# zhaoyizhou1123/OfflineRL-Kit

Measured on AMD Instinct MI355X. Metric: gradient-steps/sec (CQL, batch=256), higher is better.
Workload: dtype f32 storage / accumulate; products on split-fp16 MFMA (every operand = fp16 hi + fp16 lo plane = 22 significand bits, power-of-two operand scales folded back into the fp32 accumulators, hi*hi + hi*lo + lo*hi on v_mfma_f32_16x16x32_f16; the reference's fp32 has 24): losses and Q-values meet the 1e-4

## Files before the change

offlinerl-kit_amd/csrc/gemm.h:

```cpp
#pragma once
#include <hip/hip_runtime.h>
#include <stdint.h>

#include <algorithm>
#include <atomic>

namespace orl {

typedef float f32x4 __attribute__((ext_vector_type(4)));

#ifdef ORL_SPLIT_BF16
typedef __bf16 hx_t;
#define ORL_SPLIT_BITS 16
#define ORL_HX_ONE_BITS 0x3F80u
#define ORL_MFMA_16x16x32(a, b, c) __builtin_amdgcn_mfma_f32_16x16x32_bf16(a, b, c, 0, 0, 0)
#else
typedef _Float16 hx_t;
#define ORL_SPLIT_BITS 22
#define ORL_HX_ONE_BITS 0x3C00u
#define ORL_MFMA_16x16x32(a, b, c) __builtin_amdgcn_mfma_f32_16x16x32_f16(a, b, c, 0, 0, 0)
#endif
typedef hx_t hx4 __attribute__((ext_vector_type(4)));
typedef hx_t hx8 __attribute__((ext_vector_type(8)));
#define ORL_WSCALE 64.0f
#define ORL_WWSCALE 256.0f
#define ORL_GSCALE3 32.0f

#if defined(__HIP_DEVICE_COMPILE__) || defined(__HIPCC__)
typedef unsigned int u32x2_t __attribute__((ext_vector_type(2)));
typedef short s16x4 __attribute__((ext_vector_type(4)));
#ifdef ORL_SPLIT_BF16
#define ORL_MFMA_16x16x16(a, b, c) __builtin_amdgcn_mfma_f32_16x16x16bf16_1k(a, b, c, 0, 0, 0)
__device__ __forceinline__ void orl_split4(const f32x4& v, hx4& h, hx4& l) {
  h = __builtin_convertvector(v, hx4);
  const u32x2_t hb = *(const u32x2_t*)&h;
  f32x4 hf;
  hf[0] = __uint_as_float(hb[0] << 16); hf[1] = __uint_as_float(hb[0] & 0xffff0000u);
  hf[2] = __uint_as_float(hb[1] << 16); hf[3] = __uint_as_float(hb[1] & 0xffff0000u);
  l = __builtin_convertvector(v - hf, hx4);
}
#else
typedef _Float16 f16x4_t __attribute__((ext_vector_type(4)));
#define ORL_MFMA_16x16x16(a, b, c) __builtin_amdgcn_mfma_f32_16x16x16f16(*(const f16x4_t*)&(a), *(const f16x4_t*)&(b), c, 0, 0, 0)
__device__ __forceinline__ void orl_split4(const f32x4& v, hx4& h, hx4& l) {
  h = __builtin_convertvector(v, hx4);
#ifdef ORL_SPLIT_NO_MIX
  l = __builtin_convertvector(v - __builtin_convertvector(h, f32x4), hx4);
  return;
#endif
  const u32x2_t hb = *(const u32x2_t*)&h;
  f32x4 r;
  asm("v_fma_mix_f32 %0, %1, -1.0, %2 op_sel_hi:[1,0,0]" : "=v"(r[0]) : "v"(hb[0]), "v"(v[0]));
  asm("v_fma_mix_f32 %0, %1, -1.0, %2 op_sel:[1,0,0] op_sel_hi:[1,0,0]" : "=v"(r[1]) : "v"(hb[0]), "v"(v[1]));
  asm("v_fma_mix_f32 %0, %1, -1.0, %2 op_sel_hi:[1,0,0]" : "=v"(r[2]) : "v"(hb[1]), "v"(v[2]));
  asm("v_fma_mix_f32 %0, %1, -1.0, %2 op_sel:[1,0,0] op_sel_hi:[1,0,0]" : "=v"(r[3]) : "v"(hb[1]), "v"(v[3]));
  l = __builtin_convertvector(r, hx4);
}
#endif
__device__ __forceinline__ void orl_split1(float x, hx_t& h, hx_t& l) { h = (hx_t)x; l = (hx_t)(x - (float)h); }
__device__ __forceinline__ void orl_split4x3(const f32x4& v, hx4& h, hx4& m, hx4& l) {
  h = __builtin_convertvector(v, hx4);
#if defined(ORL_SPLIT_BF16) || defined(ORL_SPLIT_NO_MIX)
  const f32x4 r1 = v - __builtin_convertvector(h, f32x4);
  m = __builtin_convertvector(r1, hx4);
  l = __builtin_convertvector(r1 - __builtin_convertvector(m, f32x4), hx4);
#else
  const u32x2_t hb = *(const u32x2_t*)&h;
  f32x4 r1, r2;
  asm("v_fma_mix_f32 %0, %1, -1.0, %2 op_sel_hi:[1,0,0]" : "=v"(r1[0]) : "v"(hb[0]), "v"(v[0]));
  asm("v_fma_mix_f32 %0, %1, -1.0, %2 op_sel:[1,0,0] op_sel_hi:[1,0,0]" : "=v"(r1[1]) : "v"(hb[0]), "v"(v[1]));
  asm("v_fma_mix_f32 %0, %1, -1.0, %2 op_sel_hi:[1,0,0]" : "=v"(r1[2]) : "v"(hb[1]), "v"(v[2]));
  asm("v_fma_mix_f32 %0, %1, -1.0, %2 op_sel:[1,0,0] op_sel_hi:[1,0,0]" : "=v"(r1[3]) : "v"(hb[1]), "v"(v[3]));
  m = __builtin_convertvector(r1, hx4);
  const u32x2_t mb = *(const u32x2_t*)&m;
  asm("v_fma_mix_f32 %0, %1, -1.0, %2 op_sel_hi:[1,0,0]" : "=v"(r2[0]) : "v"(mb[0]), "v"(r1[0]));
  asm("v_fma_mix_f32 %0, %1, -1.0, %2 op_sel:[1,0,0] op_sel_hi:[1,0,0]" : "=v"(r2[1]) : "v"(mb[0]), "v"(r1[1]));
  asm("v_fma_mix_f32 %0, %1, -1.0, %2 op_sel_hi:[1,0,0]" : "=v"(r2[2]) : "v"(mb[1]), "v"(r1[2]));
  asm("v_fma_mix_f32 %0, %1, -1.0, %2 op_sel:[1,0,0] op_sel_hi:[1,0,0]" : "=v"(r2[3]) : "v"(mb[1]), "v"(r1[3]));
  l = __builtin_convertvector(r2, hx4);
#endif
}
__device__ __forceinline__ void orl_split1x3(float x, hx_t& h, hx_t& m, hx_t& l) {
  h = (hx_t)x;
  const float r1 = x - (float)h;
  m = (hx_t)r1;
  l = (hx_t)(r1 - (float)m);
}
__device__ __forceinline__ unsigned int orl_relu_mask4(f32x4& z) {
  unsigned int m = 0;
#pragma unroll
  for (int j = 0; j < 4; ++j) {
    const int r = max(__float_as_int(z[j]), 0);
    z[j] = __int_as_float(r);
    unsigned int b;
    asm("v_min_u32 %0, 1, %1" : "=v"(b) : "v"(r));
    m |= b << j;
  }
  return m;
}
__device__ __forceinline__ unsigned int orl_mask4(const f32x4& z) {
  unsigned int m = 0;
#pragma unroll
  for (int j = 0; j < 4; ++j) {
    const int b = min(max(__float_as_int(z[j]), 0), 1);
    m |= (unsigned int)b << j;
  }
  return m;
}
#endif

enum { P_F32 = 0, P_SPLIT = 1, P_BF16X3 = P_SPLIT, P_SPLIT3 = 2 };

enum { PA_PLAIN = 0, PA_RANK1 = 1, PA_RANK1B = 2 };
typedef unsigned int u32x4 __attribute__((ext_vector_type(4)));
enum { PB_PLAIN = 0, PB_ONES = 1 };
enum { E_PLAIN = 0, E_BIAS = 1, E_BIAS_RELU = 2, E_MASK = 3, E_WGRAD = 4,
       E_BIAS_SWISH = 5,
       E_SWISH_GRAD = 6,
       E_BIAS_LEAKY = 7,
       E_LEAKY_MASK = 8 };
#define ORL_LEAKY_SLOPE 0.01f
enum { L_SCALAR = 0, L_VECK = 1, L_BLK4 = 2, L_VECKU = 3 };

template <typename T>
struct ZView {
  T* p;
  long s0, s1;
  __host__ __device__ T* at(int z0, int z1) const { return p ? p + z0 * s0 + z1 * s1 : nullptr; }
  bool vec4() const { return (((uintptr_t)p) & 15) == 0 && !(s0 & 3) && !(s1 & 3); }
};
using ZPtr = ZView<const float>;
using ZOut = ZView<float>;
using ZBits = ZView<unsigned int>;

struct GemmP {
  ZPtr A, B;
  float* C;
  long c_s0, c_s1;
  long c_sr;
  long c_sn;
  long c_ks;
  int M, N, K;
  long a_sr, a_sk;
  long b_sr, b_sk;
  int a_rlim, b_rlim;
  int nz1;
  int ksplit;
  ZPtr rowv, colv;
  int a_trans;
  int ones_row;
  ZPtr bias;
  ZPtr aux;
  long aux_sr;
  float* bias_out;
  long bo_s0, bo_s1, bo_ks;
  float* tail_w_out; float* tail_b_out;
  long tw_s0, tw_s1, tb_s1;
  ZPtr tq_w, tq_b; float* tq_out; float* tq_part; long tq_s0, tq_s1, tq_sm, tq_ps0, tq_ps1, tq_ts;
  unsigned int* mb_out; long mb_s0, mb_s1; int mb_g;
  const unsigned int* aux_bits; long xb_s0, xb_s1; int xb_g;
  const unsigned int* a_bits; long ab_s0, ab_s1; int ab_g;
  ZPtr w0_x; long w0_xsr; int w0_in;
  float* w0_out; float* w0_bias; long w0_s0, w0_s1, w0_bs1, w0_ks, w0_sr;
  float a_scale, b_scale;
  const float* a_dscale; const float* b_dscale;
  int zmajor, nz_total;
  float* z_out;
};

#if defined(__HIP_DEVICE_COMPILE__) || defined(__HIPCC__)
__device__ __forceinline__ float orl_sigmoid(float z) { return __frcp_rn(1.0f + __expf(-z)); }
__device__ __forceinline__ float orl_swish(float z) { return z * orl_sigmoid(z); }
__device__ __forceinline__ float orl_dswish(float z) { const float s = orl_sigmoid(z); return s * (1.0f + z * (1.0f - s)); }
#endif

enum { W0_XP = 28 };

template <int WM, int WN, int MA, int NB, int TK>
struct GemmCfg {
  static constexpr int kWM = WM, kWN = WN, kMA = MA, kNB = NB, kTK = TK;
  static constexpr int TM = WM * MA * 16, TN = WN * NB * 16, NT = WM * WN * 64, PITCH = TK + 4;
  static constexpr int PITCH_H = TK + 8;
  static constexpr int LDS_FLOATS = 2 * (TM + TN) * PITCH;
  static constexpr size_t lds_bytes(int prec) {
    return prec == P_F32 ? sizeof(float) * LDS_FLOATS : (size_t)2  * (prec == P_SPLIT3 ? 3 : 2)  * (TM + TN) * PITCH_H * 2;
  }
  static constexpr size_t epi_lds_limit(int prec) { return lds_bytes(prec) > 80 * 1024 ? (size_t)160 * 1024 : lds_bytes(prec); }
  static constexpr size_t epi_lds_bytes() { return sizeof(float) * (size_t)TM * (TN + 4); }
  static_assert(TK % 16 == 0, "TK multiple of 16");
};

typedef GemmCfg<2, 4, 2, 4, 32> CfgBig;
typedef GemmCfg<2, 2, 2, 2, 32> CfgMid;
typedef GemmCfg<1, 4, 1, 1, 64> CfgSmall;
typedef GemmCfg<4, 1, 1, 1, 32> CfgTall;
typedef GemmCfg<2, 2, 4, 4, 32> CfgSq;
typedef GemmCfg<2, 4, 4, 2, 32> CfgSq8;
typedef GemmCfg<4, 2, 4, 4, 32> CfgWg;
enum { CFG_BIG = 0, CFG_MID = 1, CFG_SMALL = 2, CFG_TALL = 3, CFG_SQ = 4, CFG_SQ8 = 5, CFG_WG = 6, CFG_AUTO = -1 };

static inline int pick_cfg(int M, int N, int K, int nz) {
  if (N <= 16) return CFG_TALL;
  if (M >= 2048 && N >= 128) return ((long)M * nz >= 40000) ? CFG_SQ : CFG_BIG;
  if (M <= 32) return CFG_SMALL;
  if (K < 1024 && M >= 64 && N > 16 && N < 64 && (long)nz * ((M + 63) / 64) >= 1024) return CFG_MID;
  if (K < 1024 && M >= 64 && N >= 64) {
    if (K <= 32 && M >= 128 && N >= 128 && (long)nz * ((M + 127) / 128) * ((N + 127) / 128) >= 1024) return CFG_SQ;
    if (K >= 256 && M >= 128 && N >= 128 && (long)nz * ((M + 127) / 128) * ((N + 127) / 128) >= 256) return CFG_SQ;
    if ((long)nz * ((M + 63) / 64) * ((N + 63) / 64) >= 1024) return CFG_MID;
  }
  if (K >= 1024) return (M >= 256 && N >= 128) ? CFG_WG : ((M >= 128 && N >= 128) ? CFG_SQ : CFG_MID);
  return CFG_SMALL;
}

static inline bool aligned16(const void* p) { return (((uintptr_t)p) & 15) == 0; }

static inline int tq_fused_parts(int cfg, const GemmP& p, const float* tail_w, long tw_s0, long tw_s1) {
  const int TN = cfg == CFG_SQ8 ? CfgSq8::TN : (cfg == CFG_BIG ? CfgBig::TN : 0);
  if (!TN) return 0;
  if ((p.N & 3) || !aligned16(p.C) || (p.c_sr & 3) || (p.c_s0 & 3) || (p.c_s1 & 3) || p.c_sn != 1) return 0;
  if (!aligned16(p.bias.p) || (p.bias.s0 & 3) || (p.bias.s1 & 3)) return 0;
  if (!aligned16(tail_w) || (tw_s0 & 3) || (tw_s1 & 3)) return 0;
  return (p.N + TN - 1) / TN;
}

static inline bool mb_supported(int cfg, const GemmP& p) {
  if (cfg == CFG_TALL || (p.N & 31)) return false;
  if (!aligned16(p.C) || (p.c_sr & 3) || (p.c_s0 & 3) || (p.c_s1 & 3) || p.c_sn != 1) return false;
  return aligned16(p.bias.p) && !(p.bias.s0 & 3) && !(p.bias.s1 & 3);
}

static inline int w0_fused_slabs(const GemmP& p, int nz, int in0, long x_pitch, const void* x_ptr, long x_s0, long x_s1, int max_slab) {
  const int cfg = pick_cfg(p.M, p.N, p.K, nz);
  const int TM = cfg == CFG_SQ ? CfgSq::TM : (cfg == CFG_BIG ? CfgBig::TM : 0);
  if (!TM) return 0;
  if (in0 + 1 > W0_XP || in0 >= x_pitch || x_pitch > W0_XP || (x_pitch & 3) || !aligned16(x_ptr) || (x_s0 & 3) || (x_s1 & 3)) return 0;
  if (p.N & 3) return 0;
  if (!p.aux_bits && ((p.aux_sr & 3) || !aligned16(p.aux.p) || (p.aux.s0 & 3) || (p.aux.s1 & 3))) return 0;
  if (p.C && (!aligned16(p.C) || (p.c_sr & 3) || (p.c_s0 & 3) || (p.c_s1 & 3) || p.c_sn != 1)) return 0;
  const int tiles_m = (p.M + TM - 1) / TM;
  return tiles_m <= max_slab ? tiles_m : 0;
}

static inline int pick_loader(const ZPtr& z, long sr, long sk, int K, bool k_pad_ok, int rlim) {
  if (sk == 1 && (!aligned16(z.p) || (z.s0 & 3) || (z.s1 & 3) || (sr & 3) || !((K & 3) == 0 || k_pad_ok))) return L_VECKU;
  if (!aligned16(z.p) || (z.s0 & 3) || (z.s1 & 3)) return L_SCALAR;
  if (sk == 1 && (sr & 3) == 0 && ((K & 3) == 0 || k_pad_ok)) return L_VECK;
  if (sr == 1 && (sk & 3) == 0 && rlim >= 4 && (rlim & 3) == 0) return L_BLK4;
  return L_SCALAR;
}

static inline bool rank1_wgrad_is_fast(const GemmP& p, bool force_scalar) {
  if (force_scalar || p.a_trans != 1) return false;
  if (pick_loader(p.A, p.a_sr, p.a_sk, p.K, false, p.a_rlim) != L_BLK4) return false;
  if (pick_loader(p.B, p.b_sr, p.b_sk, p.K, false, p.b_rlim) != L_BLK4) return false;
  return aligned16(p.colv.p) && (p.colv.s0 & 3) == 0 && (p.colv.s1 & 3) == 0;
}

static inline bool rank1_bits_supported(int cfg, const GemmP& p, bool force_scalar) {
  if (force_scalar || (cfg != CFG_SQ && cfg != CFG_BIG) || p.a_trans != 0 || (p.K & 31)) return false;
  if (!aligned16(p.colv.p) || (p.colv.s0 & 3) || (p.colv.s1 & 3)) return false;
  const int lb = pick_loader(p.B, p.b_sr, p.b_sk, p.K, false, p.b_rlim);
  return lb == L_BLK4 || lb == L_VECK;
}

template <int PA, int PB, int EPI>
hipError_t launch_gemm(int cfg, const GemmP& p, int nz, hipStream_t st, bool a_kpad = false, bool force_scalar = false, int prec = P_F32);
template <int EPI>
hipError_t launch_gemm_rank1_bits(int cfg, const GemmP& p, int nz, hipStream_t st, int prec);
hipError_t launch_tune(int cfg_in, int kind, const GemmP& p, int nz, hipStream_t st);

}
```

offlinerl-kit_amd/csrc/ws_debug.hip:

```cpp
#include <hip/hip_runtime.h>

#include <cstring>
#include <string>
#include <vector>

#include "../../include/orl_engine.h"
#include "ws_gemm.h"

namespace orl {

int fail(const std::string& msg);

namespace {

typedef const WsTable& (*WsTableFn)();
static const WsTableFn WS_TABLES[] = {ws_fwd_table, ws_fwd3_table, ws_dgrad_table, ws_dgrad3_table, ws_wgrad_table, ws_wgrad3p_table};

struct WsDev {
  std::vector<void*> ptrs;
  ~WsDev() { for (void* q : ptrs) hipFree(q); }
};

enum { B_X, B_W, B_BIAS, B_TW, B_TB, B_X0, B_W0, B_B0, B_DMASK, B_ABITS, B_XBITS, B_DQ, B_WT, B_Z, B_H0, B_H1, B_W1, B_B1, B_DZ, B_GSCALE,
       B_Y, B_MB, B_MB0, B_TQ, B_TQ2, B_C, B_W0O, B_B0O, B_DW, B_DB, B_DWT, B_DBT, B_COUNT };
static const char* const WS_BUF_NAMES[B_COUNT] = {"X", "W", "bias", "tw", "tb", "X0", "W0", "b0", "dmask", "abits", "xbits", "dq", "wt", "Z", "H0", "H1",
                                                   "W1", "b1", "dZ", "gscale", "Y", "mb", "mb0", "tq", "tq2", "C", "w0_out", "b0_out", "dW", "db", "dwt", "dbt"};

static bool ws_buf_allowed(int kind, int i) {
  const bool fwd = kind == ORL_WS_FWD || kind == ORL_WS_FWD3, dg = kind == ORL_WS_DGRAD || kind == ORL_WS_DGRAD3;
  switch (i) {
    case B_X: case B_W: return fwd || dg;
    case B_BIAS: case B_TW: case B_TB: case B_DMASK: case B_Y: case B_MB: case B_MB0: case B_TQ: return fwd;
    case B_TQ2: return kind == ORL_WS_FWD3;
    case B_X0: case B_W0: case B_B0: return fwd || kind == ORL_WS_WGRAD;
    case B_XBITS: case B_Z: case B_C: case B_W0O: case B_B0O: return dg;
    case B_ABITS: case B_DQ: case B_WT: return dg || kind == ORL_WS_WGRAD;
    case B_H0: case B_DZ: case B_DW: case B_DB: return kind == ORL_WS_WGRAD || kind == ORL_WS_WGRAD3P;
    case B_H1: case B_W1: case B_B1: case B_DWT: case B_DBT: return kind == ORL_WS_WGRAD;
    default: return true;
  }
}

}
}

using namespace orl;

extern "C" {

const char* orl_debug_ws_flavour(int idx) {
  for (WsTableFn table : WS_TABLES) {
    const WsTable& t = table();
    if (idx >= 0 && idx < t.n) return t.rows[idx].name;
    idx -= t.n;
  }
  return nullptr;
}

int orl_debug_ws(orl_ws_ex* a) {
  if (!a) return fail("orl_debug_ws: null arguments");
  const int kind = a->kind, M = a->M, nz0 = a->nz0, nz1 = a->nz1, per_z = a->per_z;
  auto bad = [](const std::string& m) { return fail("orl_debug_ws: " + m); };
  if (kind < ORL_WS_FWD || kind > ORL_WS_WGRAD3P) return bad("kind must be 0..5");
  if (M < 1 || M > 4096) return bad("M must be 1..4096");
  if (M % WS_ROWS) return bad("M must be a multiple of 32 (whole row groups)");
  if (nz0 < 1 || nz1 < 1 || (long)nz0 * nz1 > 64) return bad("nz0 x nz1 must be 1..64");
  if (per_z < 1) return bad("per_z must be >= 1");
  if (per_z > M / WS_ROWS) return bad("per_z exceeds the row groups (M / 32): a workgroup would own no group");
  const int nz = nz0 * nz1, groups = M / WS_ROWS;
  const bool fwd = kind == ORL_WS_FWD || kind == ORL_WS_FWD3, dg = kind == ORL_WS_DGRAD || kind == ORL_WS_DGRAD3;
  const bool wg = kind == ORL_WS_WGRAD || kind == ORL_WS_WGRAD3P;
  if (a->f32 && (kind == ORL_WS_FWD3 || kind == ORL_WS_DGRAD3 || kind == ORL_WS_WGRAD3P)) return bad("f32 does not go with a three-plane launcher");
  if (a->np3 && kind != ORL_WS_WGRAD) return bad("np3 selects ws_wgrad_kernel<5> of launch_ws_wgrad and nothing else");
  if (a->np3 && a->f32) return bad("np3 and f32 exclude each other");

  orl_gemm_buf* bufs[B_COUNT] = {&a->X, &a->W, &a->bias, &a->tw, &a->tb, &a->X0, &a->W0, &a->b0, &a->dmask, &a->abits, &a->xbits, &a->dq, &a->wt, &a->Z,
                                 &a->H0, &a->H1, &a->W1, &a->b1, &a->dZ, &a->gscale, &a->Y, &a->mb, &a->mb0, &a->tq, &a->tq2, &a->C, &a->w0_out, &a->b0_out,
                                 &a->dW, &a->db, &a->dwt, &a->dbt};
  auto has = [&](int i) { return bufs[i]->host != nullptr; };
  for (int i = 0; i < B_COUNT; ++i)
    if (has(i) && !ws_buf_allowed(kind, i)) return bad(std::string(WS_BUF_NAMES[i]) + " does not belong to this launcher");

  std::string why;
  auto fits = [&](int i, long ext, int nslab, bool result) {
    const orl_gemm_buf& b = *bufs[i];
    const std::string name = WS_BUF_NAMES[i];
    if (!b.host) { why = name + " is required"; return false; }
    if (b.n <= 0 || b.n > (1L << 28)) { why = name + ": bad element count"; return false; }
    if (b.off < 0 || b.s0 < 0 || b.s1 < 0 || b.ks < 0 || b.pitch < 0) { why = name + ": negative offset, pitch or stride"; return false; }
    if (ext < 1) { why = name + ": empty extent"; return false; }
    if (result && ((nz0 > 1 && b.s0 < ext) || (nz1 > 1 && b.s1 < ext) || (nslab > 1 && b.ks < ext))) { why = name + ": problems or slabs of a result overlap"; return false; }
    const long last = b.off + (long)(nz0 - 1) * b.s0 + (long)(nz1 - 1) * b.s1 + (long)(nslab - 1) * b.ks + ext;
    if (last > b.n) { why = name + ": the array is shorter than its offset, strides and pitch need"; return false; }
    return true;
  };
  auto rows_fit = [&](int i, long cols, bool result) {
    if (has(i) && bufs[i]->pitch < cols) { why = std::string(WS_BUF_NAMES[i]) + ": the pitch is below the width"; return false; }
    return fits(i, (long)(M - 1) * bufs[i]->pitch + cols, 1, result);
  };
  auto narrow_fit = [&](int i) {
    if (has(i) && (bufs[i]->pitch < 1 || bufs[i]->pitch > 32)) { why = std::string(WS_BUF_NAMES[i]) + ": the pitch must be 1..32"; return false; }
    return fits(i, (long)M * bufs[i]->pitch, 1, false);
  };
  auto strided_fit = [&](int i, long sn, long sk, int nn, int nk, int nslab, bool result) {
    if (sn < 1 || sk < 1) { why = std::string(WS_BUF_NAMES[i]) + ": strides must be >= 1"; return false; }
    return fits(i, (long)(nn - 1) * sn + (long)(nk - 1) * sk + 1, nslab, result);
  };
  const bool l0 = fwd && has(B_X0), recomp = wg && has(B_X0);
  if ((l0 || recomp || (dg && has(B_W0O))) && (a->in0 < 1 || a->in0 + 1 > 32)) return bad("in0 must be 1..31 (in0 + 1 <= 32: the ones column takes a slot)");
  if (has(B_GSCALE)) {
    const orl_gemm_buf& b = a->gscale;
    if (b.n <= 0 || b.off < 0 || b.off + nz0 > b.n) return bad("gscale: one float per run (nz0) from its offset");
  }

  if (fwd) {
    const bool dgm = has(B_DMASK), tq = has(B_TQ), sy = has(B_Y);
    if (a->tq_sm < 1) return bad("tq_sm must be >= 1");
    if (has(B_TW) != tq || has(B_TB) != tq) return bad("the fused tail needs tw, tb and tq together");
    if (kind == ORL_WS_FWD3 && tq && !has(B_TQ2)) return bad("the three-plane forward writes its tail as two partial sums: tq needs tq2");
    if (has(B_TQ2) && !tq) return bad("tq2 goes with tq");
    if (dgm && (tq || l0 || has(B_BIAS) || has(B_MB) || has(B_MB0))) return bad("plain dgrad mode (dmask) has no bias, tail, fused first layer or mask output");
    if (dgm && bufs[B_DMASK]->pitch != 8) return bad("dm_g (dmask's pitch) must be 8 words");
    if (l0 != has(B_W0) || l0 != has(B_B0) || l0 != has(B_MB0)) return bad("the fused first layer needs X0, W0, b0 and mb0 together");
    if (a->x0_discard && !l0) return bad("x0_discard belongs to the fused first layer");
    if (!rows_fit(B_X, WS_K, l0) || !strided_fit(B_W, a->w_sn, a->w_sk, WS_N, WS_K, 1, false)) return bad(why);
    if (!dgm && !has(B_MB)) return bad("mb is required (the forward always emits mask words)");
    if (!dgm && (!fits(B_BIAS, WS_N, 1, false) || !rows_fit(B_MB, 8, true))) return bad(why);
    if (sy && !rows_fit(B_Y, WS_N, true)) return bad(why);
    if (tq && (!fits(B_TW, WS_N, 1, false) || !fits(B_TB, 1, 1, false) || !fits(B_TQ, (long)(M - 1) * a->tq_sm + 1, 1, true))) return bad(why);
    if (has(B_TQ2) && !fits(B_TQ2, M, 1, true)) return bad(why);
    if (dgm && !rows_fit(B_DMASK, 8, false)) return bad(why);
    if (l0) {
      if (a->in0 >= bufs[B_X0]->pitch) return bad("in0 must be below x0_pitch (the ones column needs a slot of the staged row)");
      if (bufs[B_MB0]->pitch != 8) return bad("mb0_g (mb0's pitch) must be 8 words");
      if (!narrow_fit(B_X0) || !strided_fit(B_W0, a->w0_sn, a->w0_sk, WS_N, a->in0, 1, false) || !fits(B_B0, WS_N, 1, false) || !rows_fit(B_MB0, 8, true)) return bad(why);
    }
  } else if (dg) {
    const bool plain = has(B_Z), w0 = has(B_W0O), store = has(B_C);
    if (a->dq_sm < 1) return bad("dq_sm must be >= 1");
    if (w0 == store) return bad("give either the dW0 / db0 slabs (w0_out, b0_out) or C (the stored dz0), not both and not neither");
    if (w0 != has(B_B0O)) return bad("w0_out and b0_out go together");
    if (plain && (has(B_ABITS) || has(B_DQ) || has(B_WT))) return bad("the plain flavour (Z) takes no abits, dq or wt");
    if (!has(B_XBITS) || bufs[B_XBITS]->pitch != 8) return bad("xb_g (xbits' pitch) must be 8 words");
    if (!plain && (!has(B_ABITS) || bufs[B_ABITS]->pitch != 8)) return bad("ab_g (abits' pitch) must be 8 words");
    if (!rows_fit(B_XBITS, 8, false) || !strided_fit(B_W, a->w_sn, a->w_sk, WS_N, WS_K, 1, false)) return bad(why);
    if (plain) { if (!rows_fit(B_Z, WS_K, false)) return bad(why); }
    else if (!rows_fit(B_ABITS, 8, false) || !fits(B_DQ, (long)(M - 1) * a->dq_sm + 1, 1, false) || !fits(B_WT, WS_K, 1, false)) return bad(why);
    if (w0) {
      if (!has(B_X)) return bad("X is required");
      if (a->in0 >= bufs[B_X]->pitch) return bad("in0 must be below x_pitch (the ones column needs a slot of the staged row)");
      if (a->b0_out.s0 != a->w0_out.s0 || a->b0_out.ks != a->w0_out.ks) return bad("b0_out shares w0_out's s0 and slab stride");
      if (!narrow_fit(B_X) || !strided_fit(B_W0O, a->o_sr, a->o_sc, WS_N, a->in0, per_z, true) || !fits(B_B0O, WS_N, per_z, true)) return bad(why);
    } else {
      if (has(B_X)) return bad("X belongs to the dW0 / db0 flavour");
      if (!rows_fit(B_C, WS_N, true)) return bad(why);
    }
  } else {
    const bool plain = has(B_DZ), tails = has(B_H1), derived = !tails && has(B_W1);
    if (a->dq_sm < 1) return bad("dq_sm must be >= 1");
    if (kind == ORL_WS_WGRAD3P && !plain) return bad("launch_ws_wgrad3p is the plain (materialised dZ) flavour: dZ is required");
    if (a->np3 && tails) return bad("np3 is the derived-tail flavour: it takes W1 / b1, not H1");
    if (plain && (has(B_ABITS) || has(B_DQ) || has(B_WT) || tails || has(B_W1) || has(B_B1) || has(B_DWT) || has(B_DBT))) return bad("the plain flavour (dZ) takes no abits, dq, wt, H1, W1, b1 and writes no tail gradients");
    if (recomp && !plain) return bad("X0 (recompute) belongs to the plain flavour");
    if (recomp == has(B_H0)) return bad("give either H0 or X0 / W0 / b0 (recompute)");
    if (recomp != has(B_W0) || recomp != has(B_B0)) return bad("recompute needs X0, W0 and b0 together");
    if (tails && has(B_W1)) return bad("H1 (streamed tails) and W1 (derived tails) exclude each other");
    if (has(B_W1) != has(B_B1)) return bad("W1 and b1 go together");
    if ((tails || derived) != has(B_DWT) || has(B_DWT) != has(B_DBT)) return bad("dwt and dbt go with the tail gradients (H1, or W1 / b1) and with nothing else");
    if (!plain && (!has(B_ABITS) || bufs[B_ABITS]->pitch != 8)) return bad("ab_g (abits' pitch) must be 8 words");
    if (plain) { if (!rows_fit(B_DZ, WS_K, false)) return bad(why); }
    else if (!rows_fit(B_ABITS, 8, false) || !fits(B_DQ, (long)(M - 1) * a->dq_sm + 1, 1, false) || !fits(B_WT, WS_K, 1, false)) return bad(why);
    if (recomp) {
      if (a->in0 >= bufs[B_X0]->pitch) return bad("in0 must be below x0_pitch (the ones column needs a slot of the staged row)");
      if (!narrow_fit(B_X0) || !strided_fit(B_W0, a->w0_sn, a->w0_sk, WS_N, a->in0, 1, false) || !fits(B_B0, WS_N, 1, false)) return bad(why);
    } else if (!rows_fit(B_H0, WS_N, false)) return bad(why);
    if (tails && !rows_fit(B_H1, WS_K, false)) return bad(why);
    if (derived && (!fits(B_W1, (long)WS_K * WS_N, 1, false) || !fits(B_B1, WS_K, 1, false))) return bad(why);
    if (!fits(B_DW, (long)WS_K * WS_N, per_z, true) || !fits(B_DB, WS_K, per_z, true)) return bad(why);
    if (a->db.s0 != a->dW.s0 || a->db.ks != a->dW.ks) return bad("db shares dW's s0 and slab stride");
    if (has(B_DWT)) {
      if (!fits(B_DWT, WS_K, per_z, true) || !fits(B_DBT, 1, per_z, true)) return bad(why);
      if (a->dwt.s0 != a->dW.s0 || a->dwt.ks != a->dW.ks || a->dbt.s0 != a->dW.s0 || a->dbt.ks != a->dW.ks) return bad("dwt and dbt share dW's s0 and slab stride");
    }
  }

  WsFwdP pf;
  WsDgradP pd;
  WsWgradP pw;
  auto params = [&](char* const* base, float* dump) {
    auto fp = [&](int i) -> float* { return bufs[i]->host ? (float*)base[i] + bufs[i]->off : nullptr; };
    auto zp = [&](int i) { return ZPtr{fp(i), bufs[i]->s0, bufs[i]->s1}; };
    auto zo = [&](int i) { return ZOut{fp(i), bufs[i]->s0, bufs[i]->s1}; };
    auto zb = [&](int i) { return ZBits{(unsigned int*)fp(i), bufs[i]->s0, bufs[i]->s1}; };
    memset(&pf, 0, sizeof(pf)); memset(&pd, 0, sizeof(pd)); memset(&pw, 0, sizeof(pw));
    if (fwd) {
      pf.X = zp(B_X); pf.x_pitch = (int)a->X.pitch;
      pf.W = zp(B_W); pf.w_sn = a->w_sn; pf.w_sk = a->w_sk;
      pf.bias = zp(B_BIAS);
      pf.Y = zo(B_Y); pf.y_pitch = (int)a->Y.pitch;
      pf.mb = zb(B_MB); pf.mb_g = (int)a->mb.pitch;
      pf.tw = zp(B_TW); pf.tb = zp(B_TB); pf.tq = zo(B_TQ); pf.tq_sm = a->tq_sm; pf.tq2 = zo(B_TQ2);
      pf.M = M; pf.nz1 = nz1; pf.groups = groups;
      pf.X0 = zp(B_X0); pf.x0_pitch = (int)a->X0.pitch; pf.in0 = a->in0; pf.x0_discard = a->x0_discard;
      pf.W0 = zp(B_W0); pf.w0_sn = a->w0_sn; pf.w0_sk = a->w0_sk; pf.b0 = zp(B_B0);
      pf.mb0 = zb(B_MB0); pf.mb0_g = (int)a->mb0.pitch;
      pf.dmask = zb(B_DMASK); pf.dm_g = (int)a->dmask.pitch;
      pf.f32 = a->f32; pf.gscale = fp(B_GSCALE); pf.np3 = kind == ORL_WS_FWD3; pf.dump = dump;
    } else if (dg) {
      pd.abits = zb(B_ABITS); pd.ab_g = (int)a->abits.pitch;
      pd.xbits = zb(B_XBITS); pd.xb_g = (int)a->xbits.pitch;
      pd.dq = zp(B_DQ); pd.dq_sm = a->dq_sm; pd.wt = zp(B_WT);
      pd.W = zp(B_W); pd.w_sn = a->w_sn; pd.w_sk = a->w_sk;
      pd.X = zp(B_X); pd.x_pitch = (int)a->X.pitch; pd.in0 = a->in0;
      pd.w0_out = fp(B_W0O); pd.b0_out = fp(B_B0O);
      pd.o_rs = a->w0_out.s0; pd.o_ms = a->w0_out.s1; pd.ob_ms = a->b0_out.s1; pd.o_ks = a->w0_out.ks; pd.o_sr = a->o_sr; pd.o_sc = a->o_sc;
      pd.C = zo(B_C); pd.c_pitch = (int)a->C.pitch;
      pd.Z = zp(B_Z); pd.z_pitch = (int)a->Z.pitch;
      pd.M = M; pd.nz1 = nz1; pd.groups = groups; pd.f32 = a->f32; pd.gscale = fp(B_GSCALE);
    } else {
      pw.abits = zb(B_ABITS); pw.ab_g = (int)a->abits.pitch;
      pw.dq = zp(B_DQ); pw.dq_sm = a->dq_sm;
      pw.H0 = zp(B_H0); pw.h0_pitch = (int)a->H0.pitch; pw.wt = zp(B_WT);
      pw.dW = fp(B_DW); pw.db = fp(B_DB);
      pw.o_rs = a->dW.s0; pw.o_msw = a->dW.s1; pw.o_msb = a->db.s1; pw.o_ks = a->dW.ks;
      pw.H1 = zp(B_H1); pw.h1_pitch = (int)a->H1.pitch;
      pw.dwt = fp(B_DWT); pw.dbt = fp(B_DBT); pw.o_mswt = a->dwt.s1; pw.o_msbt = a->dbt.s1;
      pw.W1 = zp(B_W1); pw.b1 = zp(B_B1);
      pw.dZ = zp(B_DZ); pw.dz_pitch = (int)a->dZ.pitch;
      pw.X0 = zp(B_X0); pw.x0_pitch = (int)a->X0.pitch; pw.in0 = a->in0;
      pw.W0 = zp(B_W0); pw.w0_sn = a->w0_sn; pw.w0_sk = a->w0_sk; pw.b0 = zp(B_B0);
      pw.M = M; pw.nz1 = nz1; pw.groups = groups; pw.f32 = a->f32; pw.np3 = a->np3; pw.gscale = fp(B_GSCALE);
    }
  };
  char* fake[B_COUNT];
  for (int i = 0; i < B_COUNT; ++i) fake[i] = (char*)(uintptr_t)4096;
  params(fake, (float*)(uintptr_t)4096);
  bool ok = false;
  int row = -1;
  const char* pred = "";
  switch (kind) {
    case ORL_WS_FWD: ok = ws_fwd_supported(pf, WS_K, WS_N) && (!l0 || ws_fwd01_supported(pf)); row = ws_fwd_flavour(pf); pred = "ws_fwd_supported / ws_fwd01_supported"; break;
    case ORL_WS_FWD3: ok = ws_fwd3_supported(pf, WS_K, WS_N); row = ws_fwd3_flavour(pf); pred = "ws_fwd3_supported"; break;
    case ORL_WS_DGRAD: ok = ws_dgrad_supported(pd, WS_K, WS_N); row = ws_dgrad_flavour(pd); pred = "ws_dgrad_supported"; break;
    case ORL_WS_DGRAD3: ok = ws_dgrad3_supported(pd, WS_K, WS_N); row = ws_dgrad3_flavour(pd); pred = "ws_dgrad3_supported"; break;
    case ORL_WS_WGRAD: ok = ws_wgrad_supported(pw, WS_K, WS_N); row = ws_wgrad_flavour(pw); pred = "ws_wgrad_supported"; break;
    default: ok = ws_wgrad3p_supported(pw, WS_K, WS_N); row = ws_wgrad3p_flavour(pw); pred = "ws_wgrad3p_supported"; break;
  }
  if (!ok) return bad(std::string("refused by ") + pred + " (M >= 256 in whole row groups, 16-byte aligned vector operands, pitches and strides that are multiples of 4, a flavour the launcher has)");
  int id = 0;
  if (row < 0) return bad("the launcher has no instantiation for these parameters");
  for (int k = 0; k < kind; ++k) id += WS_TABLES[k]().n;
  a->r_launcher = kind; a->r_flavour = id + row; a->r_lds = (int)WS_TABLES[kind]().rows[row].lds; a->r_groups = groups;
  if (a->dry_run) return 0;

  int ndev = 0;
  if (hipGetDeviceCount(&ndev) != hipSuccess || ndev == 0) return fail("no HIP device");
  WsDev dev;
  char* base[B_COUNT];
  for (int i = 0; i < B_COUNT; ++i) {
    base[i] = nullptr;
    if (!has(i)) continue;
    void* d = nullptr;
    if (hipMalloc(&d, sizeof(float) * bufs[i]->n) != hipSuccess) return fail("orl_debug_ws device: hipMalloc failed");
    dev.ptrs.push_back(d);
    base[i] = (char*)d;
    if (hipMemcpy(d, bufs[i]->host, sizeof(float) * bufs[i]->n, hipMemcpyHostToDevice) != hipSuccess) return fail("orl_debug_ws device: copy to the device failed");
  }
  float* dump = nullptr;
  if (kind == ORL_WS_FWD3) {
    if (hipMalloc((void**)&dump, sizeof(float) * (size_t)WS_DUMP_SLOTS * WS_N) != hipSuccess) return fail("orl_debug_ws device: hipMalloc failed");
    dev.ptrs.push_back(dump);
  }
  params(base, dump);
  hipStream_t st = nullptr;
  hipError_t err = hipErrorInvalidValue;
  switch (kind) {
    case ORL_WS_FWD: { WsGeom geo; geo.cus = per_z * nz; geo.one_round = true; err = launch_ws_fwd(pf, nz, st, geo); break; }
    case ORL_WS_FWD3: err = launch_ws_fwd3(pf, nz, per_z, st); break;
    case ORL_WS_DGRAD: err = launch_ws_dgrad_w0(pd, nz, per_z, st); break;
    case ORL_WS_DGRAD3: err = launch_ws_dgrad3_w0(pd, nz, per_z, st); break;
    case ORL_WS_WGRAD: err = launch_ws_wgrad(pw, nz, per_z, st); break;
    default: err = launch_ws_wgrad3p(pw, nz, per_z, st); break;
  }
  if (err != hipSuccess) return fail(std::string("orl_debug_ws device: launch: ") + hipGetErrorString(err));
  err = hipDeviceSynchronize();
  if (err != hipSuccess) return fail(std::string("orl_debug_ws device: ") + hipGetErrorString(err));
  for (int i = 0; i < B_COUNT; ++i)
    if (base[i] && hipMemcpy(bufs[i]->host, base[i], sizeof(float) * bufs[i]->n, hipMemcpyDeviceToHost) != hipSuccess) return fail("orl_debug_ws device: copy from the device failed");
  return 0;
}

}
```

offlinerl-kit_amd/csrc/ws_device.h:

```cpp
#pragma once
#include "ws_gemm.h"

namespace orl {

__device__ inline void ws_split8(const f32x4& a, const f32x4& b, hx8& h, hx8& l) {
  hx4 ha, la, hb, lb;
  orl_split4(a, ha, la);
  orl_split4(b, hb, lb);
  h = __builtin_shufflevector(ha, hb, 0, 1, 2, 3, 4, 5, 6, 7);
  l = __builtin_shufflevector(la, lb, 0, 1, 2, 3, 4, 5, 6, 7);
}

__device__ inline void ws_split8x3(const f32x4& a, const f32x4& b, hx8& h, hx8& m, hx8& l) {
  hx4 ha, ma, la, hb, mb, lb;
  orl_split4x3(a, ha, ma, la);
  orl_split4x3(b, hb, mb, lb);
  h = __builtin_shufflevector(ha, hb, 0, 1, 2, 3, 4, 5, 6, 7);
  m = __builtin_shufflevector(ma, mb, 0, 1, 2, 3, 4, 5, 6, 7);
  l = __builtin_shufflevector(la, lb, 0, 1, 2, 3, 4, 5, 6, 7);
}
__device__ __forceinline__ void ws_split8(const f32x4& a, const f32x4& b, hx8 (&pl)[2]) { ws_split8(a, b, pl[0], pl[1]); }
__device__ __forceinline__ void ws_split8(const f32x4& a, const f32x4& b, hx8 (&pl)[3]) { ws_split8x3(a, b, pl[0], pl[1], pl[2]); }

__device__ __forceinline__ int ws_a_off(int r, int kq) { return r * WS_PITCH + ((((kq >> 1) ^ (r & 15)) << 3) | ((kq & 1) << 2)); }
__device__ __forceinline__ int ws_a_frag(int s, int li, int c) { return (16 * s + li) * WS_PITCH + ((c ^ li) << 3); }

template <int CB>
__device__ __forceinline__ void ws_w_frag_load(const float* __restrict__ Wg, long w_sn, long w_sk, int ncol0, int li, int lq, f32x4 (&raw)[CB][8][2]) {
  if (w_sk == 1) {
#pragma unroll
    for (int cb = 0; cb < CB; ++cb)
#pragma unroll
      for (int ks = 0; ks < 8; ++ks) {
        const float* src = Wg + (long)(ncol0 + 16 * cb + li) * w_sn + (32 * ks + 8 * lq);
        raw[cb][ks][0] = *(const f32x4*)src; raw[cb][ks][1] = *(const f32x4*)(src + 4);
      }
  } else {
#pragma unroll
    for (int cb = 0; cb < CB; ++cb)
#pragma unroll
      for (int ks = 0; ks < 8; ++ks) {
        const float* src = Wg + (long)(ncol0 + 16 * cb + li) * w_sn + (long)(32 * ks + 8 * lq) * w_sk;
#pragma unroll
        for (int j = 0; j < 4; ++j) { raw[cb][ks][0][j] = src[(long)j * w_sk]; raw[cb][ks][1][j] = src[(long)(4 + j) * w_sk]; }
      }
  }
}

template <class P>
__device__ __forceinline__ float ws_w0_value(const P& p, const float* __restrict__ W0g, int n, int k, float bn) {
  const float w = W0g[(long)n * p.w0_sn + (long)(k < p.in0 ? k : p.in0 - 1) * p.w0_sk];
  return (k < p.in0 ? 1.f : 0.f) * w + (k == p.in0 ? 1.f : 0.f) * bn;
}
template <int NPL, class P>
__device__ __forceinline__ void ws_w0_frag(const P& p, const float* __restrict__ W0g, int n, int lq, float bn, hx8 (&pl)[NPL]) {
  f32x4 a, b;
#pragma unroll
  for (int j = 0; j < 4; ++j) {
    a[j] = ws_w0_value(p, W0g, n, 8 * lq + j, bn);
    b[j] = ws_w0_value(p, W0g, n, 8 * lq + 4 + j, bn);
  }
  ws_split8(a, b, pl);
}
template <class P>
__device__ __forceinline__ void ws_w0_frag(const P& p, const float* __restrict__ W0g, int n, int lq, float bn, f32x4 (&w)[2]) {
#pragma unroll
  for (int t = 0; t < 2; ++t)
#pragma unroll
    for (int j = 0; j < 4; ++j) w[t][j] = ws_w0_value(p, W0g, n, 16 * t + 4 * lq + j, bn);
}

template <int XI>
__device__ __forceinline__ void ws_x_index(bool on, int tid, int x0_pitch, int xe, int (&xr)[XI], int (&xc)[XI]) {
#pragma unroll
  for (int i = 0; i < XI; ++i) {
    const int e = tid + WS_NT * i;
    xr[i] = on ? e / (on ? x0_pitch : 1) : 0; xc[i] = on ? e - xr[i] * x0_pitch : 0;
    if (on && e >= xe) { xr[i] = 0; xc[i] = 32; }
  }
}
template <int XI>
__device__ __forceinline__ void ws_x_load(const float* __restrict__ X0g, int g, int xe, int tid, float (&sx)[XI]) {
#pragma unroll
  for (int i = 0; i < XI; ++i) { const int e = tid + WS_NT * i; sx[i] = X0g[(long)g * xe + (e < xe ? e : xe - 1)]; }
}
template <int NPL, int XLP, int XI>
__device__ __forceinline__ void ws_x_store(float* Xl, int buf, int in0, const int (&xr)[XI], const int (&xc)[XI], const float (&sx)[XI]) {
#pragma unroll
  for (int i = 0; i < XI; ++i) {
    const float x = (xc[i] == in0) ? 1.0f : sx[i];
    if constexpr (NPL == 0) Xl[(buf * WS_ROWS + xr[i]) * XLP + xc[i]] = x;
    else {
      hx_t* row = (hx_t*)(Xl + (buf * WS_ROWS + xr[i]) * XLP);
      const bool pad = xc[i] >= 32;
      if constexpr (NPL == 2) {
        hx_t hh, ll;
        orl_split1(x, hh, ll);
        row[pad ? 64 : xc[i]] = hh;
        row[pad ? 65 : 32 + xc[i]] = ll;
      } else {
        hx_t hh, mm, ll;
        orl_split1x3(x, hh, mm, ll);
        row[pad ? 96 : xc[i]] = hh;
        row[pad ? 97 : 32 + xc[i]] = mm;
        row[pad ? 98 : 64 + xc[i]] = ll;
      }
    }
  }
}
template <int XLP, int NPL>
__device__ __forceinline__ void ws_x_frag(const float* Xl, int xbuf, int s, int li, int lq, hx8 (&x)[NPL]) {
  const hx_t* xrow = (const hx_t*)(Xl + (xbuf * WS_ROWS + 16 * s + li) * XLP) + 8 * lq;
#pragma unroll
  for (int pl = 0; pl < NPL; ++pl) x[pl] = *(const hx8*)(xrow + 32 * pl);
}
template <int XLP>
__device__ __forceinline__ void ws_x_frag(const float* Xl, int xbuf, int s, int li, int lq, f32x4 (&x)[2]) {
  const float* xrow = Xl + (xbuf * WS_ROWS + 16 * s + li) * XLP + 4 * lq;
  x[0] = *(const f32x4*)xrow; x[1] = *(const f32x4*)(xrow + 16);
}
__device__ __forceinline__ unsigned int ws_h0_block(const hx8 (&b0)[2], const hx8 (&x)[2], f32x4& v) {
  v = (f32x4){0.f, 0.f, 0.f, 0.f};
  v = ORL_MFMA_16x16x32(b0[1], x[0], v);
  v = ORL_MFMA_16x16x32(b0[0], x[1], v);
  v = ORL_MFMA_16x16x32(b0[0], x[0], v);
  return orl_relu_mask4(v);
}
__device__ __forceinline__ unsigned int ws_h0_block(const hx8 (&b0)[3], const hx8 (&x)[3], f32x4& v) {
  v = (f32x4){0.f, 0.f, 0.f, 0.f};
  v = ORL_MFMA_16x16x32(b0[2], x[0], v);
  v = ORL_MFMA_16x16x32(b0[0], x[2], v);
  v = ORL_MFMA_16x16x32(b0[1], x[1], v);
  v = ORL_MFMA_16x16x32(b0[1], x[0], v);
  v = ORL_MFMA_16x16x32(b0[0], x[1], v);
  v = ORL_MFMA_16x16x32(b0[0], x[0], v);
  return orl_relu_mask4(v);
}
__device__ __forceinline__ unsigned int ws_h0_block(const f32x4 (&b0)[2], const f32x4 (&x)[2], f32x4& v) {
  v = (f32x4){0.f, 0.f, 0.f, 0.f};
#pragma unroll
  for (int t = 0; t < 2; ++t)
#pragma unroll
    for (int e = 0; e < 4; ++e) v = __builtin_amdgcn_mfma_f32_16x16x4f32(b0[t][e], x[t][e], v, 0, 0, 0);
  return orl_relu_mask4(v);
}

__device__ __forceinline__ unsigned int ws_pack_nibbles(const unsigned char* nb8) {
  const unsigned int* nb = (const unsigned int*)nb8;
  const unsigned int d0 = nb[0], d1 = nb[1];
  const unsigned int lo16 = (d0 & 0xFu) | ((d0 >> 4) & 0xF0u) | ((d0 >> 8) & 0xF00u) | ((d0 >> 12) & 0xF000u);
  const unsigned int hi16 = (d1 & 0xFu) | ((d1 >> 4) & 0xF0u) | ((d1 >> 8) & 0xF00u) | ((d1 >> 12) & 0xF000u);
  return lo16 | (hi16 << 16);
}
__device__ __forceinline__ float ws_tail_sum(const float* q8, float tbias) {
  float a = tbias;
#pragma unroll
  for (int w = 0; w < WS_NW; ++w) a += q8[w * WS_ROWS];
  return a;
}

__device__ __forceinline__ void ws_w0_slab_block(const WsDgradP& p, float* wo, float* bo, const f32x4& d, int c0, int lq, int n, float scale) {
#pragma unroll
  for (int r = 0; r < 4; ++r) {
    const int c = c0 + 4 * lq + r;
    if (c < p.in0) wo[(long)n * p.o_sr + (long)c * p.o_sc] = d[r] * scale;
    else if (c == p.in0) bo[n] = d[r] * scale;
  }
}

}
```

offlinerl-kit_amd/csrc/ws_dgrad.hip:

```cpp
#include "ws_device.h"

namespace orl {

template <bool W0, bool STORE, bool PLAIN = false>
__global__ __launch_bounds__(WS_NT) void ws_dgrad_w0_kernel(const WsDgradP p) {
  static_assert(WS_NW == 8 && WS_ROWS == 32, "one 32-column mask word per wave, 32-row groups");
  static_assert(!PLAIN || (W0 && !STORE), "the plain variant exists for the fused layer-0 gradient only");
  constexpr int APL = PLAIN ? 2 : 1;
  extern __shared__ __attribute__((aligned(16))) float ws_smem[];
  hx_t* Ah = (hx_t*)ws_smem;
  hx_t* XT = Ah + 2 * APL * WS_ROWS * WS_PITCH;
  float* EO = (float*)(XT + 2 * 2 * 32 * WD_XP);
  __shared__ u32x2_t mlut[16];
  const int tid = threadIdx.x, wave = tid >> 6, lane = tid & 63, li = lane & 15, lq = lane >> 4;
  const int z = blockIdx.z, z0 = z / p.nz1, z1 = z - z0 * p.nz1;
  const unsigned int* __restrict__ ab = PLAIN ? nullptr : p.abits.p + z0 * p.abits.s0 + z1 * p.abits.s1;
  const unsigned int* __restrict__ xb = p.xbits.p + z0 * p.xbits.s0 + z1 * p.xbits.s1;
  const float* __restrict__ dqg = PLAIN ? nullptr : p.dq.p + z0 * p.dq.s0 + z1 * p.dq.s1;
  const float* __restrict__ Wg = p.W.p + z0 * p.W.s0 + z1 * p.W.s1;
  const float* __restrict__ wtg = PLAIN ? nullptr : p.wt.p + z0 * p.wt.s0 + z1 * p.wt.s1;
  const float* __restrict__ Xg = p.X.p + z0 * p.X.s0 + z1 * p.X.s1;
  const float* __restrict__ Zg = PLAIN ? p.Z.p + z0 * p.Z.s0 + z1 * p.Z.s1 : nullptr;
  const int ncol0 = 32 * wave;
  const float gsc = (W0 && p.gscale) ? p.gscale[z0] : 1.f;
  constexpr float BSC = PLAIN ? ORL_WSCALE : ORL_WWSCALE;
  const float dq_sc = W0 ? gsc : 1.0f / ORL_WWSCALE;
  const float out_inv = 1.0f / (gsc * BSC);

  hx8 bh[2][8], bl[2][8];
  {
    f32x4 raw[2][8][2];
#pragma unroll
    for (int cb = 0; cb < 2; ++cb)
#pragma unroll
      for (int ks = 0; ks < 8; ++ks) {
        const int n = ncol0 + 16 * cb + li, k0 = 32 * ks + 8 * lq;
#pragma unroll
        for (int j = 0; j < 4; ++j) {
          raw[cb][ks][0][j] = Wg[(long)n * p.w_sn + (long)(k0 + j) * p.w_sk];
          raw[cb][ks][1][j] = Wg[(long)n * p.w_sn + (long)(k0 + 4 + j) * p.w_sk];
        }
      }
#pragma unroll
    for (int cb = 0; cb < 2; ++cb)
#pragma unroll
      for (int ks = 0; ks < 8; ++ks) {
        const int k0 = 32 * ks + 8 * lq;
        f32x4 t0 = (f32x4){1.f, 1.f, 1.f, 1.f}, t1 = t0;
        if (!PLAIN) { t0 = *(const f32x4*)&wtg[k0]; t1 = *(const f32x4*)&wtg[k0 + 4]; }
        ws_split8((t0 * BSC) * raw[cb][ks][0], (t1 * BSC) * raw[cb][ks][1], bh[cb][ks], bl[cb][ks]);
      }
  }
  if (W0) for (int e = tid; e < 2 * 2 * 32 * WD_XP / 2; e += WS_NT) ((unsigned int*)XT)[e] = 0u;
  if (tid < 16) mlut[tid] = (u32x2_t){((tid & 1u) | ((tid & 2u) << 15)) * ORL_HX_ONE_BITS, (((tid >> 2) & 1u) | ((tid & 8u) << 13)) * ORL_HX_ONE_BITS};
  __syncthreads();

  unsigned int sm_word;
  float sx[2];
  const int xe = W0 ? WS_ROWS * p.x_pitch : 0;
  float* __restrict__ Cg = STORE ? p.C.p + z0 * p.C.s0 + z1 * p.C.s1 : nullptr;
  int xo[2];
#pragma unroll
  for (int i = 0; i < 2; ++i) {
    const int e = tid + WS_NT * i;
    int rr = W0 ? e / (W0 ? p.x_pitch : 1) : 0, c = W0 ? e - rr * p.x_pitch : 0;
    if (e >= xe) { rr = 32; c = 0; }
    xo[i] = ((c == p.in0) ? (1 << 16) : 0) | (c * WD_XP + rr);
  }
  float sdq;
  unsigned int sxw;
  f32x4 sz[PLAIN ? 4 : 1];
  const unsigned int vo_z = PLAIN ? (unsigned int)((tid >> 6) * p.z_pitch + 4 * (tid & 63)) : 0u;
  const unsigned int vo_ab = (unsigned int)((tid >> 4) * p.ab_g + ((tid & 15) >> 1)), vo_dq = (unsigned int)((tid & 31) * (int)p.dq_sm);
  const unsigned int vo_xb = (unsigned int)(((tid >> 3) & 31) * p.xb_g + (tid & 7));
  unsigned int vo_x[2];
#pragma unroll
  for (int i = 0; i < 2; ++i) { const int e = tid + WS_NT * i; vo_x[i] = (unsigned int)(e < xe ? e : (xe > 0 ? xe - 1 : 0)); }
  auto load_group = [&](int g) __attribute__((always_inline)) {
    const long row0 = (long)g * WS_ROWS;
    if (PLAIN) {
#pragma unroll
      for (int i = 0; i < 4; ++i) sz[i] = *(const f32x4*)&(Zg + (row0 + 8 * i) * p.z_pitch)[vo_z];
    } else {
      sm_word = (ab + row0 * p.ab_g)[vo_ab];
      sdq = (dqg + row0 * p.dq_sm)[vo_dq];
    }
    sxw = (xb + row0 * p.xb_g)[vo_xb];
    if (W0) {
#pragma unroll
      for (int i = 0; i < 2; ++i) sx[i] = (Xg + (long)g * xe)[vo_x[i]];
    }
  };
  auto store_group = [&](int buf) __attribute__((always_inline)) {
    float* eo = EO + buf * (WS_ROWS + WS_NW * WS_ROWS);
    if (PLAIN) {
      hx_t* dh = Ah + (long)buf * 2 * WS_ROWS * WS_PITCH;
#pragma unroll
      for (int i = 0; i < 4; ++i) {
        const int r = (tid >> 6) + 8 * i, kq = tid & 63;
        hx4 h, l;
        orl_split4(sz[i] * gsc, h, l);
        const int o = ws_a_off(r, kq);
        *(hx4*)(dh + o) = h;
        *(hx4*)(dh + WS_ROWS * WS_PITCH + o) = l;
      }
    } else {
    const int r = tid >> 4, hw = tid & 15;
    const unsigned int bits = (sm_word >> (16 * (hw & 1))) & 0xFFFFu;
    u32x4 c0, c1;
    const u32x2_t q0 = mlut[bits & 15u], q1 = mlut[(bits >> 4) & 15u], q2 = mlut[(bits >> 8) & 15u], q3 = mlut[bits >> 12];
    c0 = (u32x4){q0[0], q0[1], q1[0], q1[1]};
    c1 = (u32x4){q2[0], q2[1], q3[0], q3[1]};
    hx_t* d = Ah + (long)buf * WS_ROWS * WS_PITCH + r * WS_PITCH;
    *(u32x4*)(d + (((2 * hw) ^ (r & 15)) << 3)) = c0;
    *(u32x4*)(d + (((2 * hw + 1) ^ (r & 15)) << 3)) = c1;
    eo[tid & 31] = sdq * dq_sc;
    }
    ((unsigned int*)eo)[WS_ROWS + (tid & 7) * WS_ROWS + ((tid >> 3) & 31)] = sxw;
    hx_t* xt = XT + (long)buf * 2 * 32 * WD_XP;
#pragma unroll
    for (int i = 0; i < 2; ++i) {
      if (W0) {
        const float x = (xo[i] >> 16) ? 1.0f : sx[i];
        hx_t hh, ll;
        orl_split1(x, hh, ll);
        xt[xo[i] & 0xFFFF] = hh;
        xt[32 * WD_XP + (xo[i] & 0xFFFF)] = ll;
      }
    }
  };

  f32x4 d2[2][2];
#pragma unroll
  for (int a = 0; a < 2; ++a)
#pragma unroll
    for (int b = 0; b < 2; ++b) d2[a][b] = (f32x4){0.f, 0.f, 0.f, 0.f};

  const int g0 = blockIdx.x, gs = gridDim.x;
  if (g0 < p.groups) {
    load_group(g0);
    store_group(0);
    if (g0 + gs < p.groups) load_group(g0 + gs);
  }
  __syncthreads();
  auto iteration = [&](int g, int it, bool steady) __attribute__((always_inline)) {
    const int buf = it & 1;
    f32x4 dq4[WS_SUB];
    unsigned int xw[WS_SUB][4];
    const float* eo = EO + buf * (WS_ROWS + WS_NW * WS_ROWS);
#pragma unroll
    for (int s = 0; s < WS_SUB; ++s) {
      dq4[s] = PLAIN ? (f32x4){1.f, 1.f, 1.f, 1.f} : *(const f32x4*)&eo[16 * s + 4 * lq];
      const u32x4 w4 = *(const u32x4*)&((const unsigned int*)eo)[WS_ROWS + wave * WS_ROWS + 16 * s + 4 * lq];
#pragma unroll
      for (int r = 0; r < 4; ++r) xw[s][r] = w4[r];
    }
    const hx_t* ah = Ah + (long)buf * APL * WS_ROWS * WS_PITCH;
    f32x4 acc[WS_SUB][2];
#pragma unroll
    for (int s = 0; s < WS_SUB; ++s)
#pragma unroll
      for (int cb = 0; cb < 2; ++cb) acc[s][cb] = (f32x4){0.f, 0.f, 0.f, 0.f};
#pragma unroll
    for (int ks = 0; ks < 8; ++ks) {
#pragma unroll
      for (int s = 0; s < WS_SUB; ++s) {
        const hx8 fa = *(const hx8*)&ah[(16 * s + li) * WS_PITCH + (((4 * ks + lq) ^ li) << 3)];
        hx8 fl;
        if (PLAIN) fl = *(const hx8*)&ah[WS_ROWS * WS_PITCH + (16 * s + li) * WS_PITCH + (((4 * ks + lq) ^ li) << 3)];
#pragma unroll
        for (int cb = 0; cb < 2; ++cb) {
          acc[s][cb] = ORL_MFMA_16x16x32(fa, bl[cb][ks], acc[s][cb]);
          if (PLAIN) acc[s][cb] = ORL_MFMA_16x16x32(fl, bh[cb][ks], acc[s][cb]);
          acc[s][cb] = ORL_MFMA_16x16x32(fa, bh[cb][ks], acc[s][cb]);
        }
      }
    }
    const hx_t* xth = XT + (long)buf * 2 * 32 * WD_XP;
    const hx_t* xtl = xth + 32 * WD_XP;
#pragma unroll
    for (int s = 0; s < WS_SUB; ++s) {
      s16x4 xh[2], xl[2];
      if (W0) {
#pragma unroll
        for (int cbk = 0; cbk < 2; ++cbk) {
          xh[cbk] = *(const s16x4*)&xth[(16 * cbk + li) * WD_XP + 16 * s + 4 * lq];
          xl[cbk] = *(const s16x4*)&xtl[(16 * cbk + li) * WD_XP + 16 * s + 4 * lq];
        }
      }
#pragma unroll
      for (int cb = 0; cb < 2; ++cb) {
        hx4 zh, zl;
#pragma unroll
        for (int r = 0; r < 4; ++r) {
          const float v = ((xw[s][r] >> (16 * cb + li)) & 1u) ? (PLAIN ? acc[s][cb][r] : acc[s][cb][r] * dq4[s][r]) : 0.f;
          if (STORE) Cg[(long)(g * WS_ROWS + 16 * s + 4 * lq + r) * p.c_pitch + ncol0 + 16 * cb + li] = v;
          hx_t hh, ll;
          orl_split1(v, hh, ll);
          zh[r] = hh; zl[r] = ll;
        }
        const s16x4 bzh = *(const s16x4*)&zh, bzl = *(const s16x4*)&zl;
#pragma unroll
        for (int cbk = 0; cbk < 2 && W0; ++cbk) {
          d2[cbk][cb] = ORL_MFMA_16x16x16(xl[cbk], bzh, d2[cbk][cb]);
          d2[cbk][cb] = ORL_MFMA_16x16x16(xh[cbk], bzl, d2[cbk][cb]);
          d2[cbk][cb] = ORL_MFMA_16x16x16(xh[cbk], bzh, d2[cbk][cb]);
        }
      }
    }
    if (steady || g + gs < p.groups) store_group(buf ^ 1);
    if (steady || g + 2 * gs < p.groups) load_group(g + 2 * gs);
    __syncthreads();
  };
  int g = g0, it = 0;
  for (; g < p.groups; g += gs, ++it) iteration(g, it, false);
  if (!W0) return;
  float* wo = p.w0_out + z0 * p.o_rs + z1 * p.o_ms + (long)blockIdx.x * p.o_ks;
  float* bo = p.b0_out + z0 * p.o_rs + z1 * p.ob_ms + (long)blockIdx.x * p.o_ks;
#pragma unroll
  for (int cbk = 0; cbk < 2; ++cbk)
#pragma unroll
    for (int cb = 0; cb < 2; ++cb) ws_w0_slab_block(p, wo, bo, d2[cbk][cb], 16 * cbk, lq, ncol0 + 16 * cb + li, out_inv);
}


template <bool W0, bool STORE, bool PLAIN = false>
__global__ __launch_bounds__(WS_NT) void ws_dgrad32_w0_kernel(const WsDgradP p) {
  static_assert(WS_NW == 8 && WS_ROWS == 32, "one 32-column mask word per wave, 32-row groups");
  static_assert(!PLAIN || (W0 && !STORE), "the plain variant exists for the fused layer-0 gradient only");
  extern __shared__ __attribute__((aligned(16))) float ws_smem[];
  float* Am = ws_smem;
  float* XT = Am + 2 * WS_ROWS * WS_K;
  float* EO = XT + 2 * 32 * WD32_XP;
  __shared__ f32x4 mlut32[16];
  const int tid = threadIdx.x, wave = tid >> 6, lane = tid & 63, li = lane & 15, lq = lane >> 4;
  const int z = blockIdx.z, z0 = z / p.nz1, z1 = z - z0 * p.nz1;
  const unsigned int* __restrict__ ab = PLAIN ? nullptr : p.abits.p + z0 * p.abits.s0 + z1 * p.abits.s1;
  const unsigned int* __restrict__ xb = p.xbits.p + z0 * p.xbits.s0 + z1 * p.xbits.s1;
  const float* __restrict__ dqg = PLAIN ? nullptr : p.dq.p + z0 * p.dq.s0 + z1 * p.dq.s1;
  const float* __restrict__ Wg = p.W.p + z0 * p.W.s0 + z1 * p.W.s1;
  const float* __restrict__ wtg = PLAIN ? nullptr : p.wt.p + z0 * p.wt.s0 + z1 * p.wt.s1;
  const float* __restrict__ Xg = p.X.p + z0 * p.X.s0 + z1 * p.X.s1;
  const float* __restrict__ Zg = PLAIN ? p.Z.p + z0 * p.Z.s0 + z1 * p.Z.s1 : nullptr;
  const int ncol0 = 32 * wave;

  f32x4 bw[2][16];
#pragma unroll
  for (int cb = 0; cb < 2; ++cb)
#pragma unroll
    for (int t = 0; t < 16; ++t) {
      const int n = ncol0 + 16 * cb + li, k0 = 16 * t + 4 * lq;
#pragma unroll
      for (int j = 0; j < 4; ++j) bw[cb][t][j] = Wg[(long)n * p.w_sn + (long)(k0 + j) * p.w_sk];
    }
  if (!PLAIN) {
#pragma unroll
    for (int cb = 0; cb < 2; ++cb)
#pragma unroll
      for (int t = 0; t < 16; ++t) bw[cb][t] *= *(const f32x4*)&wtg[16 * t + 4 * lq];
  }
  if (W0) for (int e = tid; e < 2 * 32 * WD32_XP; e += WS_NT) XT[e] = 0.f;
  if (tid < 16) mlut32[tid] = (f32x4){(float)(tid & 1), (float)((tid >> 1) & 1), (float)((tid >> 2) & 1), (float)(tid >> 3)};
  __syncthreads();

  unsigned int sm_word;
  float sx[2];
  const int xe = W0 ? WS_ROWS * p.x_pitch : 0;
  float* __restrict__ Cg = STORE ? p.C.p + z0 * p.C.s0 + z1 * p.C.s1 : nullptr;
  int xo[2];
#pragma unroll
  for (int i = 0; i < 2; ++i) {
    const int e = tid + WS_NT * i;
    int rr = W0 ? e / (W0 ? p.x_pitch : 1) : 0, c = W0 ? e - rr * p.x_pitch : 0;
    if (e >= xe) { rr = 32; c = 0; }
    xo[i] = ((c == p.in0) ? (1 << 16) : 0) | (c * WD32_XP + rr);
  }
  float sdq;
  unsigned int sxw;
  f32x4 sz[PLAIN ? 4 : 1];
  const unsigned int vo_z = PLAIN ? (unsigned int)((tid >> 6) * p.z_pitch + 4 * (tid & 63)) : 0u;
  const unsigned int vo_ab = (unsigned int)((tid >> 4) * p.ab_g + ((tid & 15) >> 1)), vo_dq = (unsigned int)((tid & 31) * (int)p.dq_sm);
  const unsigned int vo_xb = (unsigned int)(((tid >> 3) & 31) * p.xb_g + (tid & 7));
  unsigned int vo_x[2];
#pragma unroll
  for (int i = 0; i < 2; ++i) { const int e = tid + WS_NT * i; vo_x[i] = (unsigned int)(e < xe ? e : (xe > 0 ? xe - 1 : 0)); }
  auto load_group = [&](int g) __attribute__((always_inline)) {
    const long row0 = (long)g * WS_ROWS;
    if (PLAIN) {
#pragma unroll
      for (int i = 0; i < 4; ++i) sz[i] = *(const f32x4*)&(Zg + (row0 + 8 * i) * p.z_pitch)[vo_z];
    } else {
      sm_word = (ab + row0 * p.ab_g)[vo_ab];
      sdq = (dqg + row0 * p.dq_sm)[vo_dq];
    }
    sxw = (xb + row0 * p.xb_g)[vo_xb];
    if (W0) {
#pragma unroll
      for (int i = 0; i < 2; ++i) sx[i] = (Xg + (long)g * xe)[vo_x[i]];
    }
  };
  auto store_group = [&](int buf) __attribute__((always_inline)) {
    float* eo = EO + buf * (WS_ROWS + WS_NW * WS_ROWS);
    if (PLAIN) {
#pragma unroll
      for (int i = 0; i < 4; ++i) {
        const int r = (tid >> 6) + 8 * i, kq = tid & 63;
        *(f32x4*)(Am + (long)buf * WS_ROWS * WS_K + r * WS_K + ((kq ^ (r & 15)) << 2)) = sz[i];
      }
    } else {
    const int r = tid >> 4, hw = tid & 15;
    const unsigned int bits = (sm_word >> (16 * (hw & 1))) & 0xFFFFu;
    float* d = Am + (long)buf * WS_ROWS * WS_K + r * WS_K;
#pragma unroll
    for (int j = 0; j < 4; ++j)
      *(f32x4*)(d + (((4 * hw + j) ^ (r & 15)) << 2)) = mlut32[(bits >> (4 * j)) & 15u];
    eo[tid & 31] = sdq;
    }
    ((unsigned int*)eo)[WS_ROWS + (tid & 7) * WS_ROWS + ((tid >> 3) & 31)] = sxw;
    float* xt = XT + (long)buf * 32 * WD32_XP;
#pragma unroll
    for (int i = 0; i < 2; ++i)
      if (W0) xt[xo[i] & 0xFFFF] = (xo[i] >> 16) ? 1.0f : sx[i];
  };

  f32x4 d2[2][2];
#pragma unroll
  for (int a = 0; a < 2; ++a)
#pragma unroll
    for (int b = 0; b < 2; ++b) d2[a][b] = (f32x4){0.f, 0.f, 0.f, 0.f};

  const int g0 = blockIdx.x, gs = gridDim.x;
  if (g0 < p.groups) {
    load_group(g0);
    store_group(0);
    if (g0 + gs < p.groups) load_group(g0 + gs);
  }
  __syncthreads();
  auto iteration = [&](int g, int it) __attribute__((always_inline)) {
    const int buf = it & 1;
    const float* am = Am + (long)buf * WS_ROWS * WS_K;
    f32x4 acc[WS_SUB][2];
#pragma unroll
    for (int s = 0; s < WS_SUB; ++s)
#pragma unroll
      for (int cb = 0; cb < 2; ++cb) acc[s][cb] = (f32x4){0.f, 0.f, 0.f, 0.f};
#pragma unroll
    for (int t = 0; t < 16; ++t) {
      f32x4 fa[WS_SUB];
#pragma unroll
      for (int s = 0; s < WS_SUB; ++s) fa[s] = *(const f32x4*)&am[(16 * s + li) * WS_K + (((4 * t + lq) ^ li) << 2)];
#pragma unroll
      for (int e = 0; e < 4; ++e)
#pragma unroll
        for (int s = 0; s < WS_SUB; ++s)
#pragma unroll
          for (int cb = 0; cb < 2; ++cb)
            acc[s][cb] = __builtin_amdgcn_mfma_f32_16x16x4f32(fa[s][e], bw[cb][t][e], acc[s][cb], 0, 0, 0);
      __builtin_amdgcn_sched_barrier(0);
    }
    const float* eo = EO + buf * (WS_ROWS + WS_NW * WS_ROWS);
    const float* xt = XT + (long)buf * 32 * WD32_XP;
#pragma unroll
    for (int s = 0; s < WS_SUB; ++s) {
      const f32x4 dq4s = PLAIN ? (f32x4){1.f, 1.f, 1.f, 1.f} : *(const f32x4*)&eo[16 * s + 4 * lq];
      const u32x4 xws = *(const u32x4*)&((const unsigned int*)eo)[WS_ROWS + wave * WS_ROWS + 16 * s + 4 * lq];
      f32x4 xa[2];
      if (W0) {
#pragma unroll
        for (int cbk = 0; cbk < 2; ++cbk) xa[cbk] = *(const f32x4*)&xt[(16 * cbk + li) * WD32_XP + 16 * s + 4 * lq];
      }
#pragma unroll
      for (int cb = 0; cb < 2; ++cb) {
        f32x4 v;
#pragma unroll
        for (int r = 0; r < 4; ++r) {
          v[r] = ((xws[r] >> (16 * cb + li)) & 1u) ? (PLAIN ? acc[s][cb][r] : acc[s][cb][r] * dq4s[r]) : 0.f;
          if (STORE) Cg[(long)(g * WS_ROWS + 16 * s + 4 * lq + r) * p.c_pitch + ncol0 + 16 * cb + li] = v[r];
        }
#pragma unroll
        for (int cbk = 0; cbk < 2 && W0; ++cbk)
#pragma unroll
          for (int r = 0; r < 4; ++r) d2[cbk][cb] = __builtin_amdgcn_mfma_f32_16x16x4f32(xa[cbk][r], v[r], d2[cbk][cb], 0, 0, 0);
        __builtin_amdgcn_sched_barrier(0);
      }
    }
    if (g + gs < p.groups) store_group(buf ^ 1);
    if (g + 2 * gs < p.groups) load_group(g + 2 * gs);
    __syncthreads();
  };
  int g = g0, it = 0;
  for (; g < p.groups; g += gs, ++it) iteration(g, it);
  if (!W0) return;
  float* wo = p.w0_out + z0 * p.o_rs + z1 * p.o_ms + (long)blockIdx.x * p.o_ks;
  float* bo = p.b0_out + z0 * p.o_rs + z1 * p.ob_ms + (long)blockIdx.x * p.o_ks;
#pragma unroll
  for (int cbk = 0; cbk < 2; ++cbk)
#pragma unroll
    for (int cb = 0; cb < 2; ++cb) ws_w0_slab_block(p, wo, bo, d2[cbk][cb], 16 * cbk, lq, ncol0 + 16 * cb + li, 1.0f);
}

#define WS_DGRAD_ROW(NAME, KERNEL, W0, STORE, PLAIN, LDS) {NAME "<" #W0 "," #STORE "," #PLAIN ">", (const void*)KERNEL<W0, STORE, PLAIN>, LDS}
const WsTable& ws_dgrad_table() {
  static const WsFlavour rows[] = {
      WS_DGRAD_ROW("ws_dgrad", ws_dgrad_w0_kernel, 1, 0, 0, ws_dgrad_lds_bytes()), WS_DGRAD_ROW("ws_dgrad", ws_dgrad_w0_kernel, 0, 1, 0, ws_dgrad_lds_bytes()),
      WS_DGRAD_ROW("ws_dgrad", ws_dgrad_w0_kernel, 1, 0, 1, ws_dgrad_lds_bytes(true)),
      WS_DGRAD_ROW("ws_dgrad32", ws_dgrad32_w0_kernel, 1, 0, 0, ws_dgrad32_lds_bytes()), WS_DGRAD_ROW("ws_dgrad32", ws_dgrad32_w0_kernel, 0, 1, 0, ws_dgrad32_lds_bytes()),
      WS_DGRAD_ROW("ws_dgrad32", ws_dgrad32_w0_kernel, 1, 0, 1, ws_dgrad32_lds_bytes())};
  static const WsTable t = {rows, 6};
  return t;
}

int ws_dgrad_flavour(const WsDgradP& p) {
  const int row = p.Z.p ? 2 : (p.w0_out ? 0 : (p.C.p ? 1 : -1));
  return row < 0 ? -1 : row + (p.f32 ? 3 : 0);
}

hipError_t launch_ws_dgrad_w0(WsDgradP p, int nz, int per_z, hipStream_t st) {
  p.groups = p.M / WS_ROWS;
  static const hipError_t attr_err = ws_table_attrs(ws_dgrad_table());
  if (attr_err != hipSuccess) return attr_err;
  return ws_table_launch(ws_dgrad_table(), ws_dgrad_flavour(p), dim3(per_z, 1, nz), p, st);
}

}
```

offlinerl-kit_amd/csrc/ws_fwd.hip:

```cpp
#ifdef WS_FWD_WAVES16
#define WS_WAVES 16
#endif
#ifdef WS_FWD_WAVES4
#define WS_WAVES 4
#endif
#include "ws_device.h"

namespace orl {

template <bool TQ, bool L0, bool DG = false, bool SY = true, bool F32 = false, bool XS = true>
__global__ __launch_bounds__(WS_NT) void ws_fwd_kernel(const WsFwdP p) {
  extern __shared__ __attribute__((aligned(16))) float ws_smem[];
  hx_t* Ah = (hx_t*)ws_smem;
  float* Af = ws_smem;
  float* qs = ws_smem + (2 * 2 * WS_ROWS * WS_PITCH * 2) / 4;
  unsigned char* nbs = (unsigned char*)(qs + 2 * WS_NW * WS_ROWS);
  float* Xl = (float*)(nbs + 2 * WS_ROWS * WS_NBP);
  unsigned char* nbs0 = (unsigned char*)(Xl + 2 * WS_ROWS * WS_XLP);
  float* cst = (float*)((char*)ws_smem + ws_fwd_lds_bytes(L0) - sizeof(float) * 2 * WS_N);
  const int tid = threadIdx.x, wave = tid >> 6, lane = tid & 63, li = lane & 15, lq = lane >> 4;
  const int z = blockIdx.z, z0 = z / p.nz1, z1 = z - z0 * p.nz1;
  const float* __restrict__ Xg = p.X.p + z0 * p.X.s0 + z1 * p.X.s1;
  const float* __restrict__ Wg = p.W.p + z0 * p.W.s0 + z1 * p.W.s1;
  const float* __restrict__ bg = DG ? nullptr : p.bias.p + z0 * p.bias.s0 + z1 * p.bias.s1;
  float* __restrict__ Yg = p.Y.p + z0 * p.Y.s0 + z1 * p.Y.s1;
  const int ncol0 = 16 * WS_CB * wave;
  float* __restrict__ Y0g = L0 ? const_cast<float*>(Xg) : nullptr;
  const float* __restrict__ X0g = L0 ? p.X0.p + z0 * p.X0.s0 + z1 * p.X0.s1 : nullptr;

  WS_STAMP(0);
  hx8 bh[WS_CB][F32 ? 1 : 8], bl[WS_CB][F32 ? 1 : 8];
  f32x4 bw[WS_CB][F32 ? 16 : 1];
  if constexpr (F32) {
    if (p.w_sk == 1) {
#pragma unroll
      for (int cb = 0; cb < WS_CB; ++cb)
#pragma unroll
        for (int t = 0; t < 16; ++t) bw[cb][t] = *(const f32x4*)(Wg + (long)(ncol0 + 16 * cb + li) * p.w_sn + (16 * t + 4 * lq));
    } else {
#pragma unroll
      for (int cb = 0; cb < WS_CB; ++cb)
#pragma unroll
        for (int t = 0; t < 16; ++t) {
          const float* src = Wg + (long)(ncol0 + 16 * cb + li) * p.w_sn + (long)(16 * t + 4 * lq) * p.w_sk;
#pragma unroll
          for (int j = 0; j < 4; ++j) bw[cb][t][j] = src[(long)j * p.w_sk];
        }
    }
  } else {
    f32x4 raw[WS_CB][8][2];
    ws_w_frag_load(Wg, p.w_sn, p.w_sk, ncol0, li, lq, raw);
#pragma unroll
    for (int cb = 0; cb < WS_CB; ++cb)
#pragma unroll
      for (int ks = 0; ks < 8; ++ks) ws_split8(raw[cb][ks][0] * ORL_WSCALE, raw[cb][ks][1] * ORL_WSCALE, bh[cb][ks], bl[cb][ks]);
  }
  WS_STAMP(1);
  hx8 b0[WS_CB][2];
  f32x4 b0w[WS_CB][2];
  if (L0) {
    const float* __restrict__ W0g = p.W0.p + z0 * p.W0.s0 + z1 * p.W0.s1;
    const float* __restrict__ b0g = p.b0.p + z0 * p.b0.s0 + z1 * p.b0.s1;
#pragma unroll
    for (int cb = 0; cb < WS_CB; ++cb) {
      const int n = ncol0 + 16 * cb + li;
      if constexpr (F32) ws_w0_frag(p, W0g, n, lq, b0g[n], b0w[cb]); else ws_w0_frag(p, W0g, n, lq, b0g[n], b0[cb]);
    }
  }
  const float* __restrict__ twg = TQ ? p.tw.p + z0 * p.tw.s0 + z1 * p.tw.s1 : bg;
  if (!DG && tid < WS_N) { cst[tid] = bg[tid]; cst[WS_N + tid] = twg[tid]; }
  const float tbias = TQ ? (p.tb.p + z0 * p.tb.s0 + z1 * p.tb.s1)[0] : 0.f;
  const float a_sc = (DG && !F32 && p.gscale) ? p.gscale[z0] : 1.f;
  const float inv_sc = F32 ? 1.f : 1.0f / (ORL_WSCALE * a_sc);

  f32x4 st0[WS_LD];
  auto load_piece = [&](int g, f32x4 (&st)[WS_LD], int i) __attribute__((always_inline)) {
    const int idx = tid + WS_NT * i, r = idx >> 6, kq = idx & 63;
    int m = g * WS_ROWS + r; m = m < p.M ? m : p.M - 1;
    st[i] = *(const f32x4*)&Xg[(long)m * p.x_pitch + 4 * kq];
  };
  auto load_group = [&](int g, f32x4 (&st)[WS_LD]) __attribute__((always_inline)) {
#pragma unroll
    for (int i = 0; i < WS_LD; ++i) load_piece(g, st, i);
  };
  auto store_group = [&](int buf, const f32x4 (&st)[WS_LD], int i0 = 0, int i1 = WS_LD) __attribute__((always_inline)) {
    hx_t* dh = Ah + (long)buf * 2 * WS_ROWS * WS_PITCH;
    hx_t* dl = dh + WS_ROWS * WS_PITCH;
#pragma unroll
    for (int i = i0; i < i1; ++i) {
      const int idx = tid + WS_NT * i, r = idx >> 6, kq = idx & 63;
      if constexpr (F32) {
        *(f32x4*)(Af + (long)buf * WS_ROWS * WS_K + r * WS_K + ((kq ^ (r & 15)) << 2)) = st[i];
        continue;
      }
      hx4 h, l;
      if (DG) orl_split4(st[i] * a_sc, h, l); else orl_split4(st[i], h, l);
      const int o = ws_a_off(r, kq);
      *(hx4*)(dh + o) = h;
      *(hx4*)(dl + o) = l;
    }
  };

  const int xe = L0 ? WS_ROWS * p.x0_pitch : 0;
  constexpr int XI = (WS_ROWS * 32 + WS_NT - 1) / WS_NT;
  int xr[XI], xc[XI];
  float sx[XI];
  ws_x_index(L0, tid, p.x0_pitch, xe, xr, xc);
  auto loadX = [&](int g) __attribute__((always_inline)) { ws_x_load(X0g, g, xe, tid, sx); };
  auto storeX = [&](int buf) __attribute__((always_inline)) { ws_x_store<F32 ? 0 : 2, WS_XLP>(Xl, buf, p.in0, xr, xc, sx); };
  f32x4 fx32[2];
  auto prod_x = [&](int xbuf, int s, hx8 (&xa)[2]) __attribute__((always_inline)) {
    if constexpr (F32) ws_x_frag<WS_XLP>(Xl, xbuf, s, li, lq, fx32); else ws_x_frag<WS_XLP>(Xl, xbuf, s, li, lq, xa);
  };
  auto prod_block = [&](int g, int buf, int par, int s, int cb, const hx8 (&xa)[2]) __attribute__((always_inline)) {
    hx_t* dh = Ah + (long)buf * 2 * WS_ROWS * WS_PITCH;
    hx_t* dl = dh + WS_ROWS * WS_PITCH;
    const int r = 16 * s + li;
    const long m = (long)g * WS_ROWS + r;
    f32x4 v;
    unsigned int nib0;
    if constexpr (F32) nib0 = ws_h0_block(b0w[cb], fx32, v); else nib0 = ws_h0_block(b0[cb], xa, v);
    const int k = ncol0 + 16 * cb + 4 * lq;
    if constexpr (XS) *(f32x4*)&Y0g[m * p.x_pitch + k] = v;
    if constexpr (F32) {
      *(f32x4*)(Af + (long)buf * WS_ROWS * WS_K + r * WS_K + (((k >> 2) ^ (r & 15)) << 2)) = v;
    } else {
    hx4 h, l;
    orl_split4(v, h, l);
    const int o = ws_a_off(r, k >> 2);
    *(hx4*)(dh + o) = h;
    *(hx4*)(dl + o) = l;
    }
    nbs0[(par * WS_ROWS + r) * WS_NBP + (k >> 2)] = (unsigned char)nib0;
  };
  auto produce = [&](int g, int buf, int xbuf, int par) __attribute__((always_inline)) {
#pragma unroll
    for (int s = 0; s < WS_SUB; ++s) {
      hx8 xa[2];
      prod_x(xbuf, s, xa);
#pragma unroll
      for (int cb = 0; cb < WS_CB; ++cb) prod_block(g, buf, par, s, cb, xa);
    }
  };
  auto finish0 = [&](int g, int par) __attribute__((always_inline)) {
    if (tid < WS_ROWS * 8) {
      const int row = tid >> 3, wd = tid & 7;
      const unsigned int word = ws_pack_nibbles(nbs0 + (par * WS_ROWS + row) * WS_NBP + 8 * wd);
      p.mb0.p[z0 * p.mb0.s0 + z1 * p.mb0.s1 + ((long)g * WS_ROWS + row) * p.mb0_g + wd] = word;
    }
  };

  const int g0 = blockIdx.x, gs = gridDim.x;
  if (g0 >= p.groups) return;
  WS_STAMP(2);
  if (L0) {
    for (int e = tid; e < 2 * WS_ROWS * WS_XLP; e += WS_NT) Xl[e] = 0.f;
    loadX(g0);
    __syncthreads();
    storeX(0);
    if (g0 + gs < p.groups) loadX(g0 + gs);
    __syncthreads();
    produce(g0, 0, 0, 0);
    if (g0 + gs < p.groups) storeX(1);
    if (g0 + 2 * gs < p.groups) loadX(g0 + 2 * gs);
    __syncthreads();
    finish0(g0, 0);
  } else {
    load_group(g0, st0);
    store_group(0, st0);
    if (g0 + gs < p.groups) load_group(g0 + gs, st0);
    __syncthreads();
  }
  constexpr bool storeY = SY;
  auto epi_block = [&](const f32x4& a, int g, int par, int s, int cb, float& part) __attribute__((always_inline)) {
    const f32x4 bq = *(const f32x4*)&cst[ncol0 + 16 * cb + 4 * lq], twq = *(const f32x4*)&cst[WS_N + ncol0 + 16 * cb + 4 * lq];
    const int m = g * WS_ROWS + 16 * s + li;
    f32x4 v = F32 ? a + bq : a * inv_sc + bq;
    const unsigned int nib = orl_relu_mask4(v);
    if (storeY) *(f32x4*)&Yg[(long)m * p.y_pitch + ncol0 + 16 * cb + 4 * lq] = v;
    part += (v[0] * twq[0] + v[1] * twq[1]) + (v[2] * twq[2] + v[3] * twq[3]);
    nbs[(par * WS_ROWS + 16 * s + li) * WS_NBP + 4 * WS_CB * wave + 4 * cb + lq] = (unsigned char)nib;
  };
  auto epi_row = [&](int par, int s, float part) __attribute__((always_inline)) {
    if (TQ) {
      part += __shfl_xor(part, 16);
      part += __shfl_xor(part, 32);
      (qs + (par * WS_NW + wave) * WS_ROWS)[16 * s + li] = part;
    }
  };
  auto epilogue = [&](const f32x4 (&acc)[WS_SUB][WS_CB], int g, int par) __attribute__((always_inline)) {
    if (DG) {
      const unsigned int* __restrict__ dm = p.dmask.p + z0 * p.dmask.s0 + z1 * p.dmask.s1;
#pragma unroll
      for (int s = 0; s < WS_SUB; ++s) {
        const long m = (long)g * WS_ROWS + 16 * s + li;
        const unsigned int w = dm[m * p.dm_g + (ncol0 >> 5)];
#pragma unroll
        for (int cb = 0; cb < WS_CB; ++cb) {
          const unsigned int nib = w >> ((ncol0 & 31) + 16 * cb + 4 * lq);
          f32x4 v = acc[s][cb];
#pragma unroll
          for (int r = 0; r < 4; ++r) v[r] = ((nib >> r) & 1u) ? (F32 ? v[r] : v[r] * inv_sc) : 0.f;
          *(f32x4*)&Yg[m * p.y_pitch + ncol0 + 16 * cb + 4 * lq] = v;
        }
      }
      return;
    }
#pragma unroll
    for (int s = 0; s < WS_SUB; ++s) {
      float part = 0.f;
#pragma unroll
      for (int cb = 0; cb < WS_CB; ++cb) epi_block(acc[s][cb], g, par, s, cb, part);
      epi_row(par, s, part);
    }
  };
  auto finish = [&](int g, int par) __attribute__((always_inline)) {
    if (DG) return;
    if (tid < WS_ROWS * 8) {
      const int row = tid >> 3, wd = tid & 7, m = g * WS_ROWS + row;
      const unsigned int word = ws_pack_nibbles(nbs + (par * WS_ROWS + row) * WS_NBP + 8 * wd);
      p.mb.p[z0 * p.mb.s0 + z1 * p.mb.s1 + (long)m * p.mb_g + wd] = word;
    }
    if (TQ && tid < WS_ROWS) {
      const int m = g * WS_ROWS + tid;
      const float q = ws_tail_sum(qs + par * WS_NW * WS_ROWS + tid, tbias);
      p.tq.p[z0 * p.tq.s0 + z1 * p.tq.s1 + (long)m * p.tq_sm] = q;
    }
  };

  f32x4 pacc[WS_SUB][WS_CB];
  auto iteration = [&](int g, int it, f32x4 (&stn)[WS_LD], bool first, bool steady) __attribute__((always_inline)) {
    const int buf = it & 1;
    const hx_t* ah = Ah + (long)buf * 2 * WS_ROWS * WS_PITCH;
    const hx_t* al = ah + WS_ROWS * WS_PITCH;
    f32x4 acc[WS_SUB][WS_CB];
#pragma unroll
    for (int s = 0; s < WS_SUB; ++s)
#pragma unroll
      for (int cb = 0; cb < WS_CB; ++cb) acc[s][cb] = (f32x4){0.f, 0.f, 0.f, 0.f};
    const bool fine = steady && !DG;
    float fpart = 0.f;
    hx8 fxa[2];
    auto piece = [&](int ks) __attribute__((always_inline)) {
      static_assert(WS_SUB == 2 && ((WS_CB == 2 && WS_LD == 4) || (WS_CB == 1 && WS_LD == 2) || (WS_CB == 4 && WS_LD == 8)), "eight (four, sixteen) pieces");
      const int par = (it - 1) & 1;
      if constexpr (WS_CB == 4) {
#pragma unroll
        for (int h = 0; h < 2; ++h) {
          const int pc = 2 * ks + h;
          if (pc < 8) {
            const int s = pc >> 2, cb = pc & 3;
            if (cb == 0) fpart = 0.f;
            epi_block(pacc[s][cb], g - gs, par, s, cb, fpart);
            if (cb == 3) epi_row(par, s, fpart);
          } else if (L0) {
            const int s = (pc - 8) >> 2, cb = (pc - 8) & 3;
            if (cb == 0) prod_x((it + 1) & 1, s, fxa);
            prod_block(g + gs, buf ^ 1, (it + 1) & 1, s, cb, fxa);
          } else {
            store_group(buf ^ 1, stn, pc - 8, pc - 7);
            load_piece(g + 2 * gs, stn, pc - 8);
          }
        }
        return;
      }
      if constexpr (WS_CB == 1) {
        if (ks == 0 || ks == 2) {
          const int s = ks >> 1;
          fpart = 0.f;
          epi_block(pacc[s][0], g - gs, par, s, 0, fpart);
          epi_row(par, s, fpart);
        } else if (ks == 4 || ks == 6) {
          const int s = (ks - 4) >> 1;
          if (L0) {
            prod_x((it + 1) & 1, s, fxa);
            prod_block(g + gs, buf ^ 1, (it + 1) & 1, s, 0, fxa);
          } else {
            store_group(buf ^ 1, stn, s, s + 1);
            load_piece(g + 2 * gs, stn, s);
          }
        }
        return;
      }
      if (ks < 4) {
        const int s = ks >> 1, cb = ks & 1;
        if (cb == 0) fpart = 0.f;
        epi_block(pacc[s][cb], g - gs, par, s, cb, fpart);
        if (cb == 1) epi_row(par, s, fpart);
      } else if (L0) {
        const int s = (ks - 4) >> 1, cb = (ks - 4) & 1;
        if (cb == 0) prod_x((it + 1) & 1, s, fxa);
        prod_block(g + gs, buf ^ 1, (it + 1) & 1, s, cb, fxa);
      } else {
        store_group(buf ^ 1, stn, ks - 4, ks - 3);
        load_piece(g + 2 * gs, stn, ks - 4);
      }
    };
#pragma unroll
    for (int ks = 0; ks < 8; ++ks) {
      if constexpr (F32) {
        const float* af = Af + (long)buf * WS_ROWS * WS_K;
#pragma unroll
        for (int tt = 0; tt < 2; ++tt) {
          f32x4 fa[WS_SUB];
#pragma unroll
          for (int s = 0; s < WS_SUB; ++s) fa[s] = *(const f32x4*)&af[(16 * s + li) * WS_K + (((8 * ks + 4 * tt + lq) ^ li) << 2)];
#pragma unroll
          for (int e = 0; e < 4; ++e)
#pragma unroll
            for (int s = 0; s < WS_SUB; ++s)
#pragma unroll
              for (int cb = 0; cb < WS_CB; ++cb)
                acc[s][cb] = __builtin_amdgcn_mfma_f32_16x16x4f32(bw[cb][2 * ks + tt][e], fa[s][e], acc[s][cb], 0, 0, 0);
        }
      } else {
      hx8 fah2[WS_SUB], fal2[WS_SUB];
#pragma unroll
      for (int s = 0; s < WS_SUB; ++s) {
        const int o = ws_a_frag(s, li, 4 * ks + lq);
        fah2[s] = *(const hx8*)&ah[o]; fal2[s] = *(const hx8*)&al[o];
      }
#pragma unroll
      for (int s = 0; s < WS_SUB; ++s)
#pragma unroll
        for (int cb = 0; cb < WS_CB; ++cb) acc[s][cb] = ORL_MFMA_16x16x32(bl[cb][ks], fah2[s], acc[s][cb]);
#pragma unroll
      for (int s = 0; s < WS_SUB; ++s)
#pragma unroll
        for (int cb = 0; cb < WS_CB; ++cb) acc[s][cb] = ORL_MFMA_16x16x32(bh[cb][ks], fal2[s], acc[s][cb]);
#pragma unroll
      for (int s = 0; s < WS_SUB; ++s)
#pragma unroll
        for (int cb = 0; cb < WS_CB; ++cb) acc[s][cb] = ORL_MFMA_16x16x32(bh[cb][ks], fah2[s], acc[s][cb]);
      }
      if (fine) {
        piece(ks);
        __builtin_amdgcn_sched_barrier(0);
      }
    }
    if (fine) {
      if (L0) { storeX(it & 1); loadX(g + 3 * gs); }
    } else {
      if (!first) epilogue(pacc, g - gs, (it - 1) & 1);
      if (L0) {
        if (steady || g + gs < p.groups) produce(g + gs, buf ^ 1, (it + 1) & 1, (it + 1) & 1);
        if (steady || g + 2 * gs < p.groups) storeX(it & 1);
        if (steady || g + 3 * gs < p.groups) loadX(g + 3 * gs);
      } else {
        if (steady || g + gs < p.groups) store_group(buf ^ 1, stn);
        if (steady || g + 2 * gs < p.groups) load_group(g + 2 * gs, stn);
      }
    }
    __syncthreads();
    if (!first) finish(g - gs, (it - 1) & 1);
    if (L0 && (steady || g + gs < p.groups)) finish0(g + gs, (it + 1) & 1);
#pragma unroll
    for (int s = 0; s < WS_SUB; ++s)
#pragma unroll
      for (int cb = 0; cb < WS_CB; ++cb) pacc[s][cb] = acc[s][cb];
  };
  int g = g0, it = 0;
  WS_STAMP(3);
  iteration(g, it, st0, true, false);
  WS_STAMP(4);
  g += gs; ++it;
  while (g + 3 * gs < p.groups) {
    iteration(g, it, st0, false, true);
    g += gs; ++it;
  }
  while (g < p.groups) {
    iteration(g, it, st0, false, false);
    g += gs; ++it;
  }
  WS_STAMP(5);
  epilogue(pacc, g - gs, (it - 1) & 1);
  __syncthreads();
  finish(g - gs, (it - 1) & 1);
  WS_STAMP(6);
}

#define WS_FWD_ROW(TQ, L0, DG, SY, F32, XS) \
  {"ws_fwd<" #TQ "," #L0 "," #DG "," #SY "," #F32 "," #XS ">", (const void*)ws_fwd_kernel<TQ, L0, DG, SY, F32, XS>, ws_fwd_lds_bytes(L0)}
#define WS_FWD_ROWS(F32) \
  WS_FWD_ROW(1, 0, 0, 1, F32, 1), WS_FWD_ROW(0, 0, 0, 1, F32, 1), WS_FWD_ROW(1, 1, 0, 1, F32, 1), WS_FWD_ROW(0, 1, 0, 1, F32, 1), WS_FWD_ROW(0, 0, 1, 1, F32, 1), \
  WS_FWD_ROW(1, 1, 0, 0, F32, 1), WS_FWD_ROW(1, 0, 0, 0, F32, 1), WS_FWD_ROW(1, 1, 0, 0, F32, 0), WS_FWD_ROW(0, 1, 0, 1, F32, 0)
const WsTable& ws_fwd_table() {
  static const WsFlavour rows[] = {WS_FWD_ROWS(0), WS_FWD_ROWS(1)};
  static const WsTable t = {rows, 18};
  return t;
}

int ws_fwd_flavour(const WsFwdP& p) {
  const bool tq = p.tq.p != nullptr, sy = p.Y.p != nullptr, l0 = p.X0.p != nullptr;
  if (!tq && !sy) return -1;
  int row;
  if (p.dmask.p) row = 4;
  else if (l0 && p.x0_discard && !(tq && sy)) row = tq ? 7 : 8;
  else if (l0) row = tq ? (sy ? 2 : 5) : 3;
  else row = tq ? (sy ? 0 : 6) : 1;
  return row + (p.f32 ? 9 : 0);
}

hipError_t launch_ws_fwd(WsFwdP p, int nz, hipStream_t st, const WsGeom& geo) {
  p.groups = (p.M + WS_ROWS - 1) / WS_ROWS;
  const int per_z = ws_blocks_per_problem(p.groups, nz, 10, 1 << 20, geo);
  static const hipError_t attr_err = ws_table_attrs(ws_fwd_table());
  if (attr_err != hipSuccess) return attr_err;
  return ws_table_launch(ws_fwd_table(), ws_fwd_flavour(p), dim3(per_z, 1, nz), p, st);
}

}
```

offlinerl-kit_amd/csrc/ws_gemm.h:

```cpp
#pragma once
#include <hip/hip_runtime.h>
#include <cstdlib>
#include <stdint.h>

#include "gemm.h"

namespace orl {

#ifdef SB_LAB_CLOCK
#define WS_STAMP(i) do { if (p.lab_clk && threadIdx.x == 0 && blockIdx.x == 0 && blockIdx.z == 0) p.lab_clk[i] = __builtin_amdgcn_s_memtime(); } while (0)
#else
#define WS_STAMP(i) do { } while (0)
#endif

struct WsFwdP {
  ZPtr X; int x_pitch;
  ZPtr W;
  long w_sn, w_sk;
  ZPtr bias;
  ZOut Y; int y_pitch;
  ZBits mb; int mb_g;
  ZPtr tw;
  ZPtr tb;
  ZOut tq; long tq_sm;
  unsigned long long* lab_clk;
  int M, nz1, groups;
  ZPtr X0; int x0_pitch, in0;
  int x0_discard;
  ZPtr W0; long w0_sn, w0_sk;
  ZPtr b0;
  ZBits mb0; int mb0_g;
  ZBits dmask; int dm_g;
  int f32;
  const float* gscale;
  int np3;
  ZOut tq2;
  float* dump;
};
enum { WS_DUMP_SLOTS = 8192 };

#ifndef WS_WAVES
#define WS_WAVES 8
#endif
enum { WS_ROWS = 32, WS_K = 256, WS_N = 256, WS_PITCH = WS_K, WS_NW = WS_WAVES, WS_NT = 64 * WS_NW, WS_CB = WS_N / 16 / WS_NW };
enum { WS_SUB = WS_ROWS / 16, WS_LD = WS_ROWS * WS_K / 4 / WS_NT };
enum { WS_NBP = 68, WS_XLP = 36 };
enum { WF3_XLP = 52 };

struct WsFlavour { const char* name; const void* kernel; size_t lds; };
struct WsTable { const WsFlavour* rows; int n; };
static inline hipError_t ws_table_attrs(const WsTable& t) {
  hipError_t e = hipSuccess;
  for (int i = 0; i < t.n && e == hipSuccess; ++i) e = hipFuncSetAttribute(t.rows[i].kernel, hipFuncAttributeMaxDynamicSharedMemorySize, (int)t.rows[i].lds);
  return e;
}
template <class P>
static inline hipError_t ws_table_launch(const WsTable& t, int row, dim3 grid, P& p, hipStream_t st) {
  if (row < 0 || row >= t.n) return hipErrorInvalidValue;
  void* args[] = {&p};
  (void)hipLaunchKernel(t.rows[row].kernel, grid, dim3(WS_NT), args, t.rows[row].lds, st);
  return hipGetLastError();
}
static constexpr size_t ws_fwd_lds_bytes(bool l0 = false) {
  return (size_t)2 * 2 * WS_ROWS * WS_PITCH * 2 + sizeof(float) * 2 * WS_NW * WS_ROWS + 2 * WS_ROWS * WS_NBP +
         (l0 ? sizeof(float) * 2 * WS_ROWS * WS_XLP + 2 * WS_ROWS * WS_NBP : 0) + sizeof(float) * 2 * WS_N;
}

struct WsGeom { int cus = 256; bool one_round = false; };

static inline int ws_blocks_per_problem(int groups, int nz, int prologue, int cap, const WsGeom& geo) {
  const int cus = geo.cus;
  int base = cus / nz;
  if (base < 1) base = 1;
  if (base > groups) base = groups;
  if (base > cap) base = cap;
  if (geo.one_round) return base;
  int best = base;
  long best_cost = (long)((nz * (long)base + cus - 1) / cus) * (prologue + (groups + base - 1) / base);
  for (int pz = base + 1; pz <= 4 * base + 4 && pz <= groups && pz <= cap; ++pz) {
    const long cost = (long)((nz * (long)pz + cus - 1) / cus) * (prologue + (groups + pz - 1) / pz);
    if (cost < best_cost) { best_cost = cost; best = pz; }
  }
  return best;
}

const WsTable& ws_fwd_table();
int ws_fwd_flavour(const WsFwdP& p);
static inline bool ws_fwd_supported(const WsFwdP& p, int K, int N) {
  if (K != WS_K || N != WS_N || p.M < 256 || (p.M % WS_ROWS) || (!p.mb.p && !p.dmask.p)) return false;
  if (!p.X.vec4() || (p.x_pitch & 3)) return false;
  if (p.w_sk == 1 && (!p.W.vec4() || (p.w_sn & 3))) return false;
  if (p.dmask.p) { if (p.tq.p || p.X0.p || p.dm_g != 8) return false; }
  else if (!p.bias.vec4()) return false;
  if (ws_fwd_flavour(p) < 0 || (!p.Y.p && !p.mb.p)) return false;
  if (!p.Y.vec4() || (p.y_pitch & 3)) return false;
  if (p.tq.p && !p.tw.vec4()) return false;
  return true;
}

static inline bool ws_fwd01_supported(const WsFwdP& p) {
  if (!p.X0.p || !p.mb0.p || p.mb0_g != 8 || p.in0 + 1 > 32 || p.in0 >= p.x0_pitch || p.x0_pitch > 32 || WS_ROWS * p.x0_pitch > 2 * WS_NT) return false;
  return true;
}
hipError_t launch_ws_fwd(WsFwdP p, int nz, hipStream_t st, const WsGeom& geo);
static constexpr size_t ws_fwd3_lds_bytes() {
  return (size_t)2 * 3 * WS_ROWS * WS_PITCH * 2 + sizeof(float) * 2 * WS_NW * WS_ROWS + 2 * WS_ROWS * WS_NBP + sizeof(float) * 2 * WS_ROWS * WF3_XLP +
         2 * WS_ROWS * WS_NBP + sizeof(float) * 2 * WS_N;
}
const WsTable& ws_fwd3_table();
int ws_fwd3_flavour(const WsFwdP& p);
static inline bool ws_fwd3_supported(const WsFwdP& p, int K, int N) {
  if (!ws_fwd_supported(p, K, N) || (p.tq.p && !p.tq2.p)) return false;
  if (p.X0.p && (!ws_fwd01_supported(p) || !p.dump)) return false;
  return ws_fwd3_flavour(p) >= 0;
}
hipError_t launch_ws_fwd3(WsFwdP p, int nz, int per_z, hipStream_t st);

struct WsDgradP {
  ZBits abits; int ab_g;
  ZBits xbits; int xb_g;
  ZPtr dq; long dq_sm;
  ZPtr wt;
  ZPtr W; long w_sn, w_sk;
  ZPtr X; int x_pitch, in0;
  float* w0_out; float* b0_out; long o_rs, o_ms, ob_ms, o_ks; int o_sr, o_sc;
  ZOut C; int c_pitch;
  ZPtr Z; int z_pitch;
  int M, nz1, groups;
  int f32;
  const float* gscale;
};
enum { WD_XP = WS_ROWS + 4 };
static constexpr size_t ws_dgrad_lds_bytes(bool plain = false) {
  return (size_t)(plain ? 4 : 2) * WS_ROWS * WS_PITCH * 2 + (size_t)2 * 2 * 32 * WD_XP * 2 + (size_t)2 * (WS_ROWS + WS_NW * WS_ROWS) * 4;
}

enum { WD32_XP = WS_ROWS + 4 };
static constexpr size_t ws_dgrad32_lds_bytes() {
  return sizeof(float) * ((size_t)2 * WS_ROWS * WS_K + (size_t)2 * 32 * WD32_XP + (size_t)2 * (WS_ROWS + WS_NW * WS_ROWS));
}

const WsTable& ws_dgrad_table();
int ws_dgrad_flavour(const WsDgradP& p);
static inline bool ws_dgrad_supported(const WsDgradP& p, int K, int N) {
  if (K != WS_K || N != WS_N || p.M < 256 || (p.M % WS_ROWS)) return false;
  if (p.Z.p) {
    if (!p.w0_out || p.C.p || !p.xbits.p || p.xb_g != 8) return false;
    if (!p.Z.vec4() || (p.z_pitch & 3)) return false;
    return !(p.in0 + 1 > 32 || p.in0 >= p.x_pitch || p.x_pitch > 32 || WS_ROWS * p.x_pitch > 2 * WS_NT);
  }
  if (!p.abits.p || !p.xbits.p || p.ab_g != 8 || p.xb_g != 8) return false;
  if (p.w0_out && (p.in0 + 1 > 32 || p.in0 >= p.x_pitch || p.x_pitch > 32 || WS_ROWS * p.x_pitch > 2 * WS_NT)) return false;
  if (ws_dgrad_flavour(p) < 0) return false;
  return p.wt.vec4();
}
static inline int ws_dgrad_blocks(int M, int nz, int max_slab, const WsGeom& geo, int prologue = 10) {
  return ws_blocks_per_problem(M / WS_ROWS, nz, prologue, max_slab, geo);
}
hipError_t launch_ws_dgrad_w0(WsDgradP p, int nz, int per_z, hipStream_t st);
static constexpr size_t ws_dgrad3_lds_bytes(bool plain = false) {
  return (size_t)2 * (plain ? 3 : 1) * WS_ROWS * WS_PITCH * 2 + (size_t)2 * 3 * 32 * WD_XP * 2 + (size_t)2 * (WS_ROWS + WS_NW * WS_ROWS) * 4;
}
const WsTable& ws_dgrad3_table();
int ws_dgrad3_flavour(const WsDgradP& p);
static inline bool ws_dgrad3_supported(const WsDgradP& p, int K, int N) {
  return ws_dgrad_supported(p, K, N) && ws_dgrad3_flavour(p) >= 0;
}
hipError_t launch_ws_dgrad3_w0(WsDgradP p, int nz, int per_z, hipStream_t st);

struct WsWgradP {
  ZBits abits; int ab_g;
  ZPtr dq; long dq_sm;
  ZPtr H0; int h0_pitch;
  ZPtr wt;
  float *dW, *db;
  long o_rs, o_msw, o_msb, o_ks;
  ZPtr H1; int h1_pitch;
  float *dwt, *dbt; long o_mswt, o_msbt;
  ZPtr W1;
  ZPtr b1;
  ZPtr dZ; int dz_pitch;
  ZPtr X0; int x0_pitch, in0;
  ZPtr W0; long w0_sn, w0_sk;
  ZPtr b0;
  unsigned long long* lab_clk;
  int M, nz1, groups;
  int f32;
  int np3;
  const float* gscale;
};
enum { WW_IMG = WS_ROWS * WS_K };
static constexpr size_t ws_wgrad_lds_bytes(bool plain = false, bool recompute = false, bool p3 = false) {
  return (size_t)2 * ((plain || p3) ? 4 : 3) * WW_IMG * 2 + (size_t)2 * (p3 ? 3 : 2) * WS_ROWS * 16 * 2 + (recompute ? sizeof(float) * 2 * WS_ROWS * WS_XLP : 0);
}

enum { WW32_P = 272, WW32_IMG = WS_ROWS * WW32_P };
static constexpr size_t ws_wgrad32_lds_bytes(bool recompute = false) {
  return sizeof(float) * ((size_t)2 * 2 * WW32_IMG + 2 * WS_ROWS + (recompute ? 2 * WS_ROWS * WS_XLP : 0)) > sizeof(float) * 17 * WS_K
             ? sizeof(float) * ((size_t)2 * 2 * WW32_IMG + 2 * WS_ROWS + (recompute ? 2 * WS_ROWS * WS_XLP : 0)) : sizeof(float) * 17 * WS_K;
}

const WsTable& ws_wgrad_table();
int ws_wgrad_flavour(const WsWgradP& p);
static inline bool ws_wgrad_supported(const WsWgradP& p, int K, int N) {
  if (p.dZ.p) {
    if (K != WS_K || N != WS_N || p.M < 256 || (p.M % WS_ROWS)) return false;
    if (!p.dZ.vec4() || (p.dz_pitch & 3)) return false;
    if (p.X0.p) return p.W0.p && p.b0.p && p.in0 + 1 <= 32 && p.in0 < p.x0_pitch && p.x0_pitch <= 32 && WS_ROWS * p.x0_pitch <= 2 * WS_NT;
    return p.H0.vec4() && !(p.h0_pitch & 3);
  }
  if (K != WS_K || N != WS_N || p.M < 256 || (p.M % WS_ROWS) || !p.abits.p || p.ab_g != 8) return false;
  if (ws_wgrad_flavour(p) < 0) return false;
  if (!p.H0.vec4() || (p.h0_pitch & 3)) return false;
  if (!p.H1.p && p.W1.p && (!p.b1.p || !p.dwt || !p.dbt)) return false;
  if (p.H1.p && (!p.H1.vec4() || (p.h1_pitch & 3) || !p.dwt || !p.dbt)) return false;
  return p.wt.vec4();
}
hipError_t launch_ws_wgrad(WsWgradP p, int nz, int per_z, hipStream_t st);
static constexpr size_t ws_wgrad3p_lds_bytes() { return (size_t)2 * (3 * WS_ROWS * 128 + 3 * WS_ROWS * WS_K) * 2 + (size_t)WS_ROWS * 16 * 2; }
const WsTable& ws_wgrad3p_table();
int ws_wgrad3p_flavour(const WsWgradP& p);
static inline bool ws_wgrad3p_supported(const WsWgradP& p, int K, int N) {
  return ws_wgrad3p_flavour(p) >= 0 && ws_wgrad_supported(p, K, N);
}
hipError_t launch_ws_wgrad3p(WsWgradP p, int nz, int per_z, hipStream_t st);

}
```

offlinerl-kit_amd/csrc/ws_wgrad.hip:

```cpp
#include "ws_device.h"

namespace orl {

__device__ inline int ww_off(int r, int chunk, int half) { return r * WS_K + ((chunk ^ (2 * (r & 7))) << 3) + (half << 2); }

__device__ inline s16x4 ww_tr(const hx_t* img, int row0, int col0, int lane) {
  const int li = lane & 15, lq = lane >> 4, row = row0 + 4 * lq + (li >> 2), col = col0 + 4 * (li & 3);
  const hx_t* a = img + ww_off(row, col >> 3, (col >> 2) & 1);
  return __builtin_amdgcn_ds_read_tr16_b64_v4i16((s16x4 __attribute__((address_space(3)))*)a);
}

template <int MODE>
__device__ __forceinline__ void ww_finish(const WsWgradP& p, float* ws_smem, const f32x4 (&acc)[16][2], const f32x4 (&accb)[2], const f32x4& tacc,
                                          const f32x4& bacc, float dqsum, const float* __restrict__ wtg, int z0, int z1, int ncol0, float inv = 1.0f) {
  constexpr bool TAILS = (MODE == 1);
  const int tid = threadIdx.x, wave = tid >> 6, lane = tid & 63, li = lane & 15, lq = lane >> 4;
  const long so = z0 * p.o_rs + (long)blockIdx.x * p.o_ks;
  float* dW = p.dW + so + z1 * p.o_msw;
  float* db = p.db + so + z1 * p.o_msb;
  if (MODE == 2) {
    const float* __restrict__ W1g = p.W1.p + z0 * p.W1.s0 + z1 * p.W1.s1;
    float* red = ws_smem;
#pragma unroll
    for (int kb2 = 0; kb2 < 16; kb2 += 2) {
      float wa[2][4], wb[2][4];
#pragma unroll
      for (int h = 0; h < 2; ++h)
#pragma unroll
        for (int r = 0; r < 4; ++r) {
          const int o = 16 * (kb2 + h) + 4 * lq + r;
          wa[h][r] = W1g[(long)o * WS_N + ncol0 + li];
          wb[h][r] = W1g[(long)o * WS_N + ncol0 + 16 + li];
        }
#pragma unroll
      for (int h = 0; h < 2; ++h)
#pragma unroll
        for (int r = 0; r < 4; ++r) {
          const int o = 16 * (kb2 + h) + 4 * lq + r;
          float t = (wa[h][r] * acc[kb2 + h][0][r] + wb[h][r] * acc[kb2 + h][1][r]) * inv;
          t += __builtin_bit_cast(float, __builtin_amdgcn_update_dpp(0, __builtin_bit_cast(int, t), 0xB1, 0xF, 0xF, false));
          t += __builtin_bit_cast(float, __builtin_amdgcn_update_dpp(0, __builtin_bit_cast(int, t), 0x4E, 0xF, 0xF, false));
          t += __builtin_bit_cast(float, __builtin_amdgcn_update_dpp(0, __builtin_bit_cast(int, t), 0x141, 0xF, 0xF, false));
          t += __builtin_bit_cast(float, __builtin_amdgcn_update_dpp(0, __builtin_bit_cast(int, t), 0x140, 0xF, 0xF, false));
          if (li == 0) red[wave * WS_K + o] = t;
        }
    }
  }
  if (MODE == 3) {
#pragma unroll
    for (int kb = 0; kb < 16; ++kb)
#pragma unroll
      for (int nb = 0; nb < 2; ++nb)
#pragma unroll
        for (int r = 0; r < 4; ++r) dW[(long)(16 * kb + 4 * lq + r) * WS_N + ncol0 + 16 * nb + li] = acc[kb][nb][r] * inv;
    if (li == 0) {
#pragma unroll
      for (int x = 0; x < 2; ++x) {
        const int k0 = 16 * (2 * wave + x) + 4 * lq;
#pragma unroll
        for (int r = 0; r < 4; ++r) db[k0 + r] = accb[x][r] * inv;
      }
    }
    return;
  }
#pragma unroll
  for (int kb = 0; kb < 16; ++kb) {
    const f32x4 w4 = *(const f32x4*)&wtg[16 * kb + 4 * lq];
#pragma unroll
    for (int nb = 0; nb < 2; ++nb)
#pragma unroll
      for (int r = 0; r < 4; ++r) dW[(long)(16 * kb + 4 * lq + r) * WS_N + ncol0 + 16 * nb + li] = (w4[r] * inv) * acc[kb][nb][r];
  }
  if (MODE == 2) {
    float* red = ws_smem;
    if (li == 0) {
#pragma unroll
      for (int x = 0; x < 2; ++x)
#pragma unroll
        for (int r = 0; r < 4; ++r) red[8 * WS_K + 16 * (2 * wave + x) + 4 * lq + r] = accb[x][r] * inv;
    }
    if (lane == 0) red[9 * WS_K + wave] = dqsum;
    __syncthreads();
    if (tid < WS_K) {
      float a = 0.f;
#pragma unroll
      for (int w = 0; w < 8; ++w) a += red[w * WS_K + tid];
      const float gs1 = red[8 * WS_K + tid];
      p.dwt[so + z1 * p.o_mswt + tid] = a + (p.b1.p + z0 * p.b1.s0 + z1 * p.b1.s1)[tid] * gs1;
      db[tid] = wtg[tid] * gs1;
    }
    if (tid == 0) {
      float a = 0.f;
#pragma unroll
      for (int w = 0; w < 8; ++w) a += red[9 * WS_K + w];
      p.dbt[so + z1 * p.o_msbt] = a;
    }
    return;
  }
  if (!TAILS) {
    if (li == 0) {
#pragma unroll
      for (int x = 0; x < 2; ++x) {
        const int k0 = 16 * (2 * wave + x) + 4 * lq;
#pragma unroll
        for (int r = 0; r < 4; ++r) db[k0 + r] = wtg[k0 + r] * (accb[x][r] * inv);
      }
    }
    return;
  }
  float* red = ws_smem;
  *(f32x4*)&red[(tid >> 6) * WS_K + 4 * (tid & 63)] = tacc;
  *(f32x4*)&red[(8 + (tid >> 6)) * WS_K + 4 * (tid & 63)] = bacc;
  if ((tid & 63) == 0) red[16 * WS_K + (tid >> 6)] = dqsum;
  __syncthreads();
  if (tid < WS_K) {
    float a = 0.f, b = 0.f;
#pragma unroll
    for (int w = 0; w < 8; ++w) { a += red[w * WS_K + tid]; b += red[(8 + w) * WS_K + tid]; }
    p.dwt[so + z1 * p.o_mswt + tid] = a;
    db[tid] = wtg[tid] * b;
  }
  if (tid == 0) {
    float a = 0.f;
#pragma unroll
    for (int w = 0; w < 8; ++w) a += red[16 * WS_K + w];
    p.dbt[so + z1 * p.o_msbt] = a;
  }
}

template <int MODE>
__global__ __launch_bounds__(WS_NT) void ws_wgrad_kernel(const WsWgradP p) {
  static_assert(WS_NW == 8 && WS_ROWS == 32, "8 waves x 32 columns, 32-row groups");
  constexpr bool TAILS = (MODE == 1), PLAIN = (MODE == 3 || MODE == 4), RECOMP = (MODE == 4), P3 = (MODE == 5);
  constexpr int NPL = (PLAIN || P3) ? 4 : 3;
  constexpr int DQP = P3 ? 3 : 2;
  extern __shared__ __attribute__((aligned(16))) float ws_smem[];
  hx_t* img = (hx_t*)ws_smem;
  __shared__ u32x2_t mlut[16];
  const int tid = threadIdx.x, wave = tid >> 6, lane = tid & 63, li = lane & 15, lq = lane >> 4;
  const int z = blockIdx.z, z0 = z / p.nz1, z1 = z - z0 * p.nz1;
  const unsigned int* __restrict__ ab = PLAIN ? nullptr : p.abits.p + z0 * p.abits.s0 + z1 * p.abits.s1;
  const float* __restrict__ dqg = PLAIN ? nullptr : p.dq.p + z0 * p.dq.s0 + z1 * p.dq.s1;
  const float* __restrict__ H0g = p.H0.p + z0 * p.H0.s0 + z1 * p.H0.s1;
  const float* __restrict__ wtg = PLAIN ? nullptr : p.wt.p + z0 * p.wt.s0 + z1 * p.wt.s1;
  const int ncol0 = 32 * wave;
  const float gsc = p.gscale ? p.gscale[z0] : 1.f;

  WS_STAMP(0);
  f32x4 acc[16][2], accb[2];
#pragma unroll
  for (int kb = 0; kb < 16; ++kb)
#pragma unroll
    for (int nb = 0; nb < 2; ++nb) acc[kb][nb] = (f32x4){0.f, 0.f, 0.f, 0.f};
  accb[0] = accb[1] = (f32x4){0.f, 0.f, 0.f, 0.f};

  f32x4 s0[4];
  f32x4 s1[(TAILS || PLAIN) ? 4 : 1];
  f32x4 tacc = (f32x4){0.f, 0.f, 0.f, 0.f}, bacc = (f32x4){0.f, 0.f, 0.f, 0.f};
  float dqsum = 0.f;
  const float* __restrict__ H1g = TAILS ? p.H1.p + z0 * p.H1.s0 + z1 * p.H1.s1 : (PLAIN ? p.dZ.p + z0 * p.dZ.s0 + z1 * p.dZ.s1 : nullptr);
  const int h1_pitch = PLAIN ? p.dz_pitch : p.h1_pitch;
  float sdq[4];
  unsigned int sm_word;
  hx_t* dqimg = img + 2 * NPL * WW_IMG;
  float* Xl = (float*)(dqimg + 2 * DQP * WS_ROWS * 16);
  const float* __restrict__ X0g = RECOMP ? p.X0.p + z0 * p.X0.s0 + z1 * p.X0.s1 : nullptr;
  hx8 b0[2][2];
  if (RECOMP) {
    const float* __restrict__ W0g = p.W0.p + z0 * p.W0.s0 + z1 * p.W0.s1;
    const float* __restrict__ b0g = p.b0.p + z0 * p.b0.s0 + z1 * p.b0.s1;
#pragma unroll
    for (int cb = 0; cb < 2; ++cb) ws_w0_frag(p, W0g, ncol0 + 16 * cb + li, lq, b0g[ncol0 + 16 * cb + li], b0[cb]);
  }
  const int xe = RECOMP ? WS_ROWS * p.x0_pitch : 0;
  int xr[2], xc[2];
  float sx[2];
  ws_x_index(RECOMP, tid, p.x0_pitch, xe, xr, xc);
  auto loadX = [&](int g) __attribute__((always_inline)) { ws_x_load(X0g, g, xe, tid, sx); };
  auto storeX = [&](int xbuf) __attribute__((always_inline)) { ws_x_store<2, WS_XLP>(Xl, xbuf, p.in0, xr, xc, sx); };
  hx8 xa[2];
  auto prod_x = [&](int xbuf, int s) __attribute__((always_inline)) { ws_x_frag<WS_XLP>(Xl, xbuf, s, li, lq, xa); };
  auto prod_block = [&](int buf, int s, int cb) __attribute__((always_inline)) {
    hx_t* gh = img + (long)buf * NPL * WW_IMG + (NPL - 2) * WW_IMG;
    hx_t* gl = gh + WW_IMG;
    f32x4 v;
    ws_h0_block(b0[cb], xa, v);
    hx4 h, l;
    orl_split4(v, h, l);
    const int k = ncol0 + 16 * cb + 4 * lq;
    const int o = ww_off(16 * s + li, k >> 3, (k >> 2) & 1);
    *(hx4*)(gh + o) = h;
    *(hx4*)(gl + o) = l;
  };
  const unsigned int vo_h0 = (unsigned int)((tid >> 6) * p.h0_pitch + 4 * (tid & 63));
  const unsigned int vo_h1 = (TAILS || PLAIN) ? (unsigned int)((tid >> 6) * h1_pitch + 4 * (tid & 63)) : 0u;
  const unsigned int vo_dq = (unsigned int)((tid >> 6) * (int)p.dq_sm);
  const unsigned int vo_ab = (unsigned int)((tid >> 4) * p.ab_g + ((tid & 15) >> 1));
  auto load_piece = [&](int g, int i) __attribute__((always_inline)) {
    const long row0 = (long)g * WS_ROWS + 8 * i;
    if (!RECOMP) s0[i] = *(const f32x4*)&(H0g + row0 * p.h0_pitch)[vo_h0];
    if (TAILS || PLAIN) s1[i] = *(const f32x4*)&(H1g + row0 * h1_pitch)[vo_h1];
    if (!PLAIN) sdq[i] = (dqg + row0 * p.dq_sm)[vo_dq];
  };
  auto load_mask = [&](int g) __attribute__((always_inline)) {
    if (!PLAIN) sm_word = (ab + (long)g * WS_ROWS * p.ab_g)[vo_ab];
  };
  auto load_group = [&](int g) __attribute__((always_inline)) {
    load_mask(g);
#pragma unroll
    for (int i = 0; i < 4; ++i) load_piece(g, i);
  };
  auto store_mask = [&](int buf) __attribute__((always_inline)) {
    if (PLAIN) return;
    hx_t* mi = img + (long)buf * NPL * WW_IMG;
    const int r = tid >> 4, hw = tid & 15;
    const unsigned int bits = (sm_word >> (16 * (hw & 1))) & 0xFFFFu;
    u32x4 c0, c1;
    const u32x2_t q0 = mlut[bits & 15u], q1 = mlut[(bits >> 4) & 15u], q2 = mlut[(bits >> 8) & 15u], q3 = mlut[bits >> 12];
    c0 = (u32x4){q0[0], q0[1], q1[0], q1[1]};
    c1 = (u32x4){q2[0], q2[1], q3[0], q3[1]};
    *(u32x4*)(mi + ww_off(r, 2 * hw, 0)) = c0;
    *(u32x4*)(mi + ww_off(r, 2 * hw + 1, 0)) = c1;
  };
  auto store_piece = [&](int buf, int i) __attribute__((always_inline)) {
    hx_t* gh = img + (long)buf * NPL * WW_IMG + (NPL - 2) * WW_IMG;
    hx_t* gl = gh + WW_IMG;
    const int idx = tid + WS_NT * i, r = idx >> 6, kq = idx & 63;
    hx4 h, l;
    const int o = ww_off(r, kq >> 1, kq & 1);
    if (PLAIN) {
      if (!RECOMP) {
        orl_split4(s0[i], h, l);
        *(hx4*)(gh + o) = h;
        *(hx4*)(gl + o) = l;
      }
      hx_t* zh = img + (long)buf * NPL * WW_IMG;
      orl_split4(s1[i] * gsc, h, l);
      *(hx4*)(zh + o) = h;
      *(hx4*)(zh + WW_IMG + o) = l;
      return;
    }
    const float dqs = sdq[i] * gsc;
    if (P3) {
      hx4 m;
      hx_t* g3 = img + (long)buf * NPL * WW_IMG + WW_IMG;
      orl_split4x3(s0[i] * dqs, h, m, l);
      *(hx4*)(g3 + o) = h;
      *(hx4*)(g3 + WW_IMG + o) = m;
      *(hx4*)(g3 + 2 * WW_IMG + o) = l;
      if (kq == 0) {
        hx_t hh, mm, ll;
        orl_split1x3(dqs, hh, mm, ll);
        hx_t* dqi = dqimg + (long)buf * DQP * WS_ROWS * 16;
        dqi[r * 16] = hh; dqi[WS_ROWS * 16 + r * 16] = mm; dqi[2 * WS_ROWS * 16 + r * 16] = ll;
        dqsum += sdq[i];
      }
      return;
    }
    orl_split4(s0[i] * dqs, h, l);
    *(hx4*)(gh + o) = h;
    *(hx4*)(gl + o) = l;
    if (TAILS) {
#pragma unroll
      for (int j = 0; j < 4; ++j) { tacc[j] += sdq[i] * s1[i][j]; bacc[j] += s1[i][j] > 0.f ? sdq[i] : 0.f; }
      dqsum += sdq[i];
    } else if (kq == 0) {
      hx_t hh, ll;
      orl_split1(dqs, hh, ll);
      hx_t* dqi = dqimg + (long)buf * 2 * WS_ROWS * 16;
      dqi[r * 16] = hh; dqi[WS_ROWS * 16 + r * 16] = ll;
      if (MODE == 2) dqsum += sdq[i];
    }
  };
  auto store_group = [&](int buf) __attribute__((always_inline)) {
    store_mask(buf);
#pragma unroll
    for (int i = 0; i < 4; ++i) store_piece(buf, i);
  };
  if (!TAILS) for (int e = tid; e < 2 * DQP * WS_ROWS * 16 / 2; e += WS_NT) ((unsigned int*)dqimg)[e] = 0u;
  if (PLAIN) {
    __syncthreads();
    if (tid < 2 * WS_ROWS) (dqimg + (long)(tid >> 5) * 2 * WS_ROWS * 16)[(tid & 31) * 16] = (hx_t)1.0f;
  }
  if (tid < 16) mlut[tid] = (u32x2_t){((tid & 1u) | ((tid & 2u) << 15)) * ORL_HX_ONE_BITS, (((tid >> 2) & 1u) | ((tid & 8u) << 13)) * ORL_HX_ONE_BITS};
  if (RECOMP) for (int e = tid; e < 2 * WS_ROWS * WS_XLP; e += WS_NT) Xl[e] = 0.f;
  __syncthreads();

  const int g0 = blockIdx.x, gs = gridDim.x;
  WS_STAMP(1);
  if (RECOMP && g0 < p.groups) {
    loadX(g0);
    storeX(0);
    if (g0 + gs < p.groups) loadX(g0 + gs);
    __syncthreads();
#pragma unroll
    for (int s = 0; s < 2; ++s) {
      prod_x(0, s);
#pragma unroll
      for (int cb = 0; cb < 2; ++cb) prod_block(0, s, cb);
    }
    if (g0 + gs < p.groups) storeX(1);
  }
  if (g0 < p.groups) {
    load_group(g0);
    store_group(0);
    if (g0 + gs < p.groups) load_group(g0 + gs);
  }
  __syncthreads();
  auto iteration = [&](int g, int it, bool steady) __attribute__((always_inline)) {
    const int buf = it & 1;
    const bool more = steady || g + gs < p.groups, more2 = steady || g + 2 * gs < p.groups;
    const hx_t* mi = img + (long)buf * NPL * WW_IMG;
    const hx_t* ml = mi + WW_IMG;
    const hx_t* gh = mi + (P3 ? 1 : NPL - 2) * WW_IMG;
    const hx_t* gl = gh + (P3 ? 2 : 1) * WW_IMG;
    const hx_t* gm = gh + WW_IMG;
    const hx_t* dqi = dqimg + (long)buf * DQP * WS_ROWS * 16;
    {
      auto cat = [](s16x4 x, s16x4 y) __attribute__((always_inline)) {
        hx8 r;
        *(s16x4*)&r = x; *((s16x4*)&r + 1) = y;
        return r;
      };
      hx8 bh[2], bl[2], bm[2];
#pragma unroll
      for (int nb = 0; nb < 2; ++nb) {
        bh[nb] = cat(ww_tr(gh, 0, ncol0 + 16 * nb, lane), ww_tr(gh, 16, ncol0 + 16 * nb, lane));
        bl[nb] = cat(ww_tr(gl, 0, ncol0 + 16 * nb, lane), ww_tr(gl, 16, ncol0 + 16 * nb, lane));
        if (P3) bm[nb] = cat(ww_tr(gm, 0, ncol0 + 16 * nb, lane), ww_tr(gm, 16, ncol0 + 16 * nb, lane));
      }
      const int dro0 = (4 * lq + (li >> 2)) * 16 + 4 * (li & 3), dro1 = dro0 + 16 * 16;
      typedef s16x4 __attribute__((address_space(3))) * lds_s16x4;
#pragma unroll
      for (int kp = 0; kp < 8; ++kp) {
        const int kb0 = 2 * kp, kb1 = kb0 + 1;
        const hx8 a0 = cat(ww_tr(mi, 0, 16 * kb0, lane), ww_tr(mi, 16, 16 * kb0, lane));
        const hx8 a1 = cat(ww_tr(mi, 0, 16 * kb1, lane), ww_tr(mi, 16, 16 * kb1, lane));
#pragma unroll
        for (int nb = 0; nb < 2; ++nb) acc[kb0][nb] = ORL_MFMA_16x16x32(a0, bl[nb], acc[kb0][nb]);
#pragma unroll
        for (int nb = 0; nb < 2; ++nb) acc[kb1][nb] = ORL_MFMA_16x16x32(a1, bl[nb], acc[kb1][nb]);
        if (P3) {
#pragma unroll
          for (int nb = 0; nb < 2; ++nb) acc[kb0][nb] = ORL_MFMA_16x16x32(a0, bm[nb], acc[kb0][nb]);
#pragma unroll
          for (int nb = 0; nb < 2; ++nb) acc[kb1][nb] = ORL_MFMA_16x16x32(a1, bm[nb], acc[kb1][nb]);
        }
        if (PLAIN) {
          const hx8 l0 = cat(ww_tr(ml, 0, 16 * kb0, lane), ww_tr(ml, 16, 16 * kb0, lane));
          const hx8 l1 = cat(ww_tr(ml, 0, 16 * kb1, lane), ww_tr(ml, 16, 16 * kb1, lane));
#pragma unroll
          for (int nb = 0; nb < 2; ++nb) acc[kb0][nb] = ORL_MFMA_16x16x32(l0, bh[nb], acc[kb0][nb]);
#pragma unroll
          for (int nb = 0; nb < 2; ++nb) acc[kb1][nb] = ORL_MFMA_16x16x32(l1, bh[nb], acc[kb1][nb]);
        }
#pragma unroll
        for (int nb = 0; nb < 2; ++nb) acc[kb0][nb] = ORL_MFMA_16x16x32(a0, bh[nb], acc[kb0][nb]);
#pragma unroll
        for (int nb = 0; nb < 2; ++nb) acc[kb1][nb] = ORL_MFMA_16x16x32(a1, bh[nb], acc[kb1][nb]);
        if (!TAILS && kp == 7) {
          hx8 bdh, bdl, bdm;
          bdh = cat(__builtin_amdgcn_ds_read_tr16_b64_v4i16((lds_s16x4)(dqi + dro0)), __builtin_amdgcn_ds_read_tr16_b64_v4i16((lds_s16x4)(dqi + dro1)));
          bdl = cat(__builtin_amdgcn_ds_read_tr16_b64_v4i16((lds_s16x4)(dqi + (DQP - 1) * WS_ROWS * 16 + dro0)),
                    __builtin_amdgcn_ds_read_tr16_b64_v4i16((lds_s16x4)(dqi + (DQP - 1) * WS_ROWS * 16 + dro1)));
          if (P3) bdm = cat(__builtin_amdgcn_ds_read_tr16_b64_v4i16((lds_s16x4)(dqi + WS_ROWS * 16 + dro0)),
                            __builtin_amdgcn_ds_read_tr16_b64_v4i16((lds_s16x4)(dqi + WS_ROWS * 16 + dro1)));
          const hx8 c0 = cat(ww_tr(mi, 0, 32 * wave, lane), ww_tr(mi, 16, 32 * wave, lane));
          const hx8 c1 = cat(ww_tr(mi, 0, 32 * wave + 16, lane), ww_tr(mi, 16, 32 * wave + 16, lane));
          if (PLAIN) {
            const hx8 e0 = cat(ww_tr(ml, 0, 32 * wave, lane), ww_tr(ml, 16, 32 * wave, lane));
            const hx8 e1 = cat(ww_tr(ml, 0, 32 * wave + 16, lane), ww_tr(ml, 16, 32 * wave + 16, lane));
            accb[0] = ORL_MFMA_16x16x32(e0, bdh, accb[0]);
            accb[1] = ORL_MFMA_16x16x32(e1, bdh, accb[1]);
          } else {
            accb[0] = ORL_MFMA_16x16x32(c0, bdl, accb[0]);
            accb[1] = ORL_MFMA_16x16x32(c1, bdl, accb[1]);
            if (P3) {
              accb[0] = ORL_MFMA_16x16x32(c0, bdm, accb[0]);
              accb[1] = ORL_MFMA_16x16x32(c1, bdm, accb[1]);
            }
          }
          accb[0] = ORL_MFMA_16x16x32(c0, bdh, accb[0]);
          accb[1] = ORL_MFMA_16x16x32(c1, bdh, accb[1]);
        }
        if (kp < 4) {
          if (more) store_piece(buf ^ 1, kp);
          if (more2) load_piece(g + 2 * gs, kp);
        }
        if (RECOMP) {
          if (kp == 0 && more2) loadX(g + 2 * gs);
          if (kp >= 4 && more) {
            if (!(kp & 1)) prod_x(buf ^ 1, (kp - 4) >> 1);
            prod_block(buf ^ 1, (kp - 4) >> 1, kp & 1);
          }
          if (kp == 7 && more2) storeX(buf);
        }
        if (kp == 5) {
          if (more) store_mask(buf ^ 1);
          if (more2) load_mask(g + 2 * gs);
        }
      }
    }
    __syncthreads();
  };
  int g = g0, it = 0;
  WS_STAMP(2);
  for (; MODE != 1 && g + 2 * gs < p.groups; g += gs, ++it) iteration(g, it, true);
  for (; g < p.groups; g += gs, ++it) iteration(g, it, false);
  WS_STAMP(3);

  ww_finish<(MODE == 4 ? 3 : (MODE == 5 ? 2 : MODE))>(p, ws_smem, acc, accb, tacc, bacc, dqsum, wtg, z0, z1, ncol0, 1.0f / gsc);
  WS_STAMP(4);
}


template <int MODE>
__global__ __launch_bounds__(WS_NT) void ws_wgrad32_kernel(const WsWgradP p) {
  static_assert(WS_NW == 8 && WS_ROWS == 32, "8 waves x 32 columns, 32-row groups");
  constexpr bool TAILS = (MODE == 1), PLAIN = (MODE == 3 || MODE == 4), RECOMP = (MODE == 4);
  extern __shared__ __attribute__((aligned(16))) float ws_smem[];
  float* img = ws_smem;
  float* dqs = img + 2 * 2 * WW32_IMG;
  float* Xl = dqs + 2 * WS_ROWS;
  __shared__ f32x4 mlut[16];
  const int tid = threadIdx.x, wave = tid >> 6, lane = tid & 63, li = lane & 15, lq = lane >> 4;
  const int z = blockIdx.z, z0 = z / p.nz1, z1 = z - z0 * p.nz1;
  const unsigned int* __restrict__ ab = PLAIN ? nullptr : p.abits.p + z0 * p.abits.s0 + z1 * p.abits.s1;
  const float* __restrict__ dqg = PLAIN ? nullptr : p.dq.p + z0 * p.dq.s0 + z1 * p.dq.s1;
  const float* __restrict__ H0g = p.H0.p + z0 * p.H0.s0 + z1 * p.H0.s1;
  const float* __restrict__ wtg = PLAIN ? nullptr : p.wt.p + z0 * p.wt.s0 + z1 * p.wt.s1;
  const float* __restrict__ H1g = TAILS ? p.H1.p + z0 * p.H1.s0 + z1 * p.H1.s1 : (PLAIN ? p.dZ.p + z0 * p.dZ.s0 + z1 * p.dZ.s1 : nullptr);
  const int h1_pitch = PLAIN ? p.dz_pitch : p.h1_pitch;
  const int ncol0 = 32 * wave;

  f32x4 acc[16][2], accb[2];
#pragma unroll
  for (int kb = 0; kb < 16; ++kb)
#pragma unroll
    for (int nb = 0; nb < 2; ++nb) acc[kb][nb] = (f32x4){0.f, 0.f, 0.f, 0.f};
  accb[0] = accb[1] = (f32x4){0.f, 0.f, 0.f, 0.f};
  f32x4 s0[4];
  f32x4 s1[(TAILS || PLAIN) ? 4 : 1];
  f32x4 tacc = (f32x4){0.f, 0.f, 0.f, 0.f}, bacc = (f32x4){0.f, 0.f, 0.f, 0.f};
  float dqsum = 0.f;
  float sdq[4];
  unsigned int sm_word;
  const float* __restrict__ X0g = RECOMP ? p.X0.p + z0 * p.X0.s0 + z1 * p.X0.s1 : nullptr;
  f32x4 b0w[2][2];
  if (RECOMP) {
    const float* __restrict__ W0g = p.W0.p + z0 * p.W0.s0 + z1 * p.W0.s1;
    const float* __restrict__ b0g = p.b0.p + z0 * p.b0.s0 + z1 * p.b0.s1;
#pragma unroll
    for (int cb = 0; cb < 2; ++cb) ws_w0_frag(p, W0g, ncol0 + 16 * cb + li, lq, b0g[ncol0 + 16 * cb + li], b0w[cb]);
  }
  const int xe = RECOMP ? WS_ROWS * p.x0_pitch : 0;
  int xr[2], xc[2];
  float sx[2];
  ws_x_index(RECOMP, tid, p.x0_pitch, xe, xr, xc);
  auto loadX = [&](int g) __attribute__((always_inline)) { ws_x_load(X0g, g, xe, tid, sx); };
  auto storeX = [&](int xbuf) __attribute__((always_inline)) { ws_x_store<0, WS_XLP>(Xl, xbuf, p.in0, xr, xc, sx); };
  f32x4 fx32[2];
  auto prod_x = [&](int xbuf, int s) __attribute__((always_inline)) { ws_x_frag<WS_XLP>(Xl, xbuf, s, li, lq, fx32); };
  auto prod_block = [&](int buf, int s, int cb) __attribute__((always_inline)) {
    float* gi = img + (long)buf * 2 * WW32_IMG + WW32_IMG;
    f32x4 v;
    ws_h0_block(b0w[cb], fx32, v);
    *(f32x4*)(gi + (16 * s + li) * WW32_P + ncol0 + 16 * cb + 4 * lq) = v;
  };
  const unsigned int vo_h0 = (unsigned int)((tid >> 6) * p.h0_pitch + 4 * (tid & 63));
  const unsigned int vo_h1 = (TAILS || PLAIN) ? (unsigned int)((tid >> 6) * h1_pitch + 4 * (tid & 63)) : 0u;
  const unsigned int vo_dq = (unsigned int)((tid >> 6) * (int)p.dq_sm);
  const unsigned int vo_ab = (unsigned int)((tid >> 4) * p.ab_g + ((tid & 15) >> 1));
  auto load_piece = [&](int g, int i) __attribute__((always_inline)) {
    const long row0 = (long)g * WS_ROWS + 8 * i;
    if (!RECOMP) s0[i] = *(const f32x4*)&(H0g + row0 * p.h0_pitch)[vo_h0];
    if (TAILS || PLAIN) s1[i] = *(const f32x4*)&(H1g + row0 * h1_pitch)[vo_h1];
    if (!PLAIN) sdq[i] = (dqg + row0 * p.dq_sm)[vo_dq];
  };
  auto load_mask = [&](int g) __attribute__((always_inline)) {
    if (!PLAIN) sm_word = (ab + (long)g * WS_ROWS * p.ab_g)[vo_ab];
  };
  auto load_group = [&](int g) __attribute__((always_inline)) {
    load_mask(g);
#pragma unroll
    for (int i = 0; i < 4; ++i) load_piece(g, i);
  };
  auto store_mask = [&](int buf) __attribute__((always_inline)) {
    if (PLAIN) return;
    float* mi = img + (long)buf * 2 * WW32_IMG;
    const int r = tid >> 4, hw = tid & 15;
    const unsigned int bits = (sm_word >> (16 * (hw & 1))) & 0xFFFFu;
#pragma unroll
    for (int j = 0; j < 4; ++j) *(f32x4*)(mi + r * WW32_P + 16 * hw + 4 * j) = mlut[(bits >> (4 * j)) & 15u];
  };
  auto store_piece = [&](int buf, int i) __attribute__((always_inline)) {
    float* gi = img + (long)buf * 2 * WW32_IMG + WW32_IMG;
    const int idx = tid + WS_NT * i, r = idx >> 6, kq = idx & 63;
    if (PLAIN) {
      if (!RECOMP) *(f32x4*)(gi + r * WW32_P + 4 * kq) = s0[i];
      *(f32x4*)(gi - WW32_IMG + r * WW32_P + 4 * kq) = s1[i];
      return;
    }
    *(f32x4*)(gi + r * WW32_P + 4 * kq) = s0[i] * sdq[i];
    if (TAILS) {
#pragma unroll
      for (int j = 0; j < 4; ++j) { tacc[j] += sdq[i] * s1[i][j]; bacc[j] += s1[i][j] > 0.f ? sdq[i] : 0.f; }
      dqsum += sdq[i];
    } else if (kq == 0) {
      dqs[buf * WS_ROWS + r] = sdq[i];
      if (MODE == 2) dqsum += sdq[i];
    }
  };
  auto store_group = [&](int buf) __attribute__((always_inline)) {
    store_mask(buf);
#pragma unroll
    for (int i = 0; i < 4; ++i) store_piece(buf, i);
  };

  if (threadIdx.x < 16) mlut[threadIdx.x] = (f32x4){(float)(threadIdx.x & 1u), (float)((threadIdx.x >> 1) & 1u), (float)((threadIdx.x >> 2) & 1u), (float)(threadIdx.x >> 3)};
  if (RECOMP) for (int e = tid; e < 2 * WS_ROWS * WS_XLP; e += WS_NT) Xl[e] = 0.f;
  __syncthreads();
  const int g0 = blockIdx.x, gs = gridDim.x;
  if (RECOMP && g0 < p.groups) {
    loadX(g0);
    storeX(0);
    if (g0 + gs < p.groups) loadX(g0 + gs);
    __syncthreads();
#pragma unroll
    for (int s = 0; s < 2; ++s) {
      prod_x(0, s);
#pragma unroll
      for (int cb = 0; cb < 2; ++cb) prod_block(0, s, cb);
    }
    if (g0 + gs < p.groups) storeX(1);
  }
  if (g0 < p.groups) {
    load_group(g0);
    store_group(0);
    if (g0 + gs < p.groups) load_group(g0 + gs);
  }
  __syncthreads();
  auto iteration = [&](int g, int it, bool steady) __attribute__((always_inline)) {
    const int buf = it & 1;
    const bool more = steady || g + gs < p.groups, more2 = steady || g + 2 * gs < p.groups;
    const float* mi = img + (long)buf * 2 * WW32_IMG;
    const float* gi = mi + WW32_IMG;
    const float* dqb = dqs + buf * WS_ROWS;
    const int ro = lq * WW32_P + li;
    float bg[2][8], bd[8];
#pragma unroll
    for (int st = 0; st < 8; ++st) {
#pragma unroll
      for (int nb = 0; nb < 2; ++nb) bg[nb][st] = gi[4 * st * WW32_P + ro + ncol0 + 16 * nb];
      if (!TAILS) { const float d = PLAIN ? 1.0f : dqb[4 * st + lq]; bd[st] = li == 0 ? d : 0.f; }
    }
#pragma unroll
    for (int kp = 0; kp < 8; ++kp) {
      const int kb0 = 2 * kp, kb1 = kb0 + 1;
      float a0[8], a1[8];
#pragma unroll
      for (int st = 0; st < 8; ++st) { a0[st] = mi[4 * st * WW32_P + ro + 16 * kb0]; a1[st] = mi[4 * st * WW32_P + ro + 16 * kb1]; }
#pragma unroll
      for (int st = 0; st < 8; ++st) {
#pragma unroll
        for (int nb = 0; nb < 2; ++nb) acc[kb0][nb] = __builtin_amdgcn_mfma_f32_16x16x4f32(a0[st], bg[nb][st], acc[kb0][nb], 0, 0, 0);
#pragma unroll
        for (int nb = 0; nb < 2; ++nb) acc[kb1][nb] = __builtin_amdgcn_mfma_f32_16x16x4f32(a1[st], bg[nb][st], acc[kb1][nb], 0, 0, 0);
      }
      if (!TAILS && kp == 7) {
        float c0[8], c1[8];
#pragma unroll
        for (int st = 0; st < 8; ++st) { c0[st] = mi[4 * st * WW32_P + ro + 32 * wave]; c1[st] = mi[4 * st * WW32_P + ro + 32 * wave + 16]; }
#pragma unroll
        for (int st = 0; st < 8; ++st) {
          accb[0] = __builtin_amdgcn_mfma_f32_16x16x4f32(c0[st], bd[st], accb[0], 0, 0, 0);
          accb[1] = __builtin_amdgcn_mfma_f32_16x16x4f32(c1[st], bd[st], accb[1], 0, 0, 0);
        }
      }
      if (kp < 4) {
        if (more) store_piece(buf ^ 1, kp);
        if (more2) load_piece(g + 2 * gs, kp);
      }
      if (RECOMP) {
        if (kp == 0 && more2) loadX(g + 2 * gs);
        if (kp >= 4 && more) {
          if (!(kp & 1)) prod_x(buf ^ 1, (kp - 4) >> 1);
          prod_block(buf ^ 1, (kp - 4) >> 1, kp & 1);
        }
        if (kp == 7 && more2) storeX(buf);
      }
      if (kp == 5) {
        if (more) store_mask(buf ^ 1);
        if (more2) load_mask(g + 2 * gs);
      }
    }
    __syncthreads();
  };
  int g = g0, it = 0;
  for (; MODE != 1 && g + 2 * gs < p.groups; g += gs, ++it) iteration(g, it, true);
  for (; g < p.groups; g += gs, ++it) iteration(g, it, false);
  ww_finish<(MODE == 4 ? 3 : MODE)>(p, ws_smem, acc, accb, tacc, bacc, dqsum, wtg, z0, z1, ncol0);
}

#define WS_WGRAD_ROW(MODE) {"ws_wgrad<" #MODE ">", (const void*)ws_wgrad_kernel<MODE>, ws_wgrad_lds_bytes(MODE == 3 || MODE == 4, MODE == 4, MODE == 5)}
#define WS_WGRAD32_ROW(MODE) {"ws_wgrad32<" #MODE ">", (const void*)ws_wgrad32_kernel<MODE>, ws_wgrad32_lds_bytes(MODE == 4)}
const WsTable& ws_wgrad_table() {
  static const WsFlavour rows[] = {WS_WGRAD_ROW(0), WS_WGRAD_ROW(1), WS_WGRAD_ROW(2), WS_WGRAD_ROW(3), WS_WGRAD_ROW(4), WS_WGRAD_ROW(5),
                                                WS_WGRAD32_ROW(0), WS_WGRAD32_ROW(1), WS_WGRAD32_ROW(2), WS_WGRAD32_ROW(3), WS_WGRAD32_ROW(4)};
  static const WsTable t = {rows, 11};
  return t;
}

int ws_wgrad_flavour(const WsWgradP& p) {
  if (p.dZ.p) return (p.X0.p ? 4 : 3) + (p.f32 ? 6 : 0);
  if (p.np3) return (p.H1.p || !p.W1.p) ? -1 : 5;
  return (p.H1.p ? 1 : (p.W1.p ? 2 : 0)) + (p.f32 ? 6 : 0);
}

hipError_t launch_ws_wgrad(WsWgradP p, int nz, int per_z, hipStream_t st) {
  p.groups = p.M / WS_ROWS;
  static const hipError_t attr_err = ws_table_attrs(ws_wgrad_table());
  if (attr_err != hipSuccess) return attr_err;
  return ws_table_launch(ws_wgrad_table(), ws_wgrad_flavour(p), dim3(per_z, 1, nz), p, st);
}

}
```

Measured before the change: 54520.

## Precompute per-lane byte offsets for global and LDS addressing in workspace GEMM kernels

Replaces per-iteration index arithmetic in the fwd, dgrad and wgrad kernels with 32-bit per-lane byte offsets computed once and combined with uniform bases through inline-asm-pinned global pointers, and with XOR-swizzled LDS byte offsets. Single-value fp16 splits now use a v_fma_mix residual. Guards reject problems whose 32-bit spans would overflow. The goal is fewer VALU address instructions and possibly fewer VGPRs, at the cost of more complex addressing that must match the old swizzles exactly.

```diff
diff --git a/offlinerl-kit_amd/csrc/gemm.h b/offlinerl-kit_amd/csrc/gemm.h
--- a/offlinerl-kit_amd/csrc/gemm.h
+++ b/offlinerl-kit_amd/csrc/gemm.h
@@ -58,6 +58,17 @@
 }
 #endif
 __device__ __forceinline__ void orl_split1(float x, hx_t& h, hx_t& l) { h = (hx_t)x; l = (hx_t)(x - (float)h); }
+__device__ __forceinline__ void orl_split1m(float x, hx_t& h, hx_t& l) {
+#if defined(ORL_SPLIT_BF16) || defined(ORL_SPLIT_NO_MIX)
+  orl_split1(x, h, l);
+#else
+  h = (hx_t)x;
+  const unsigned int hb = (unsigned int)__builtin_bit_cast(unsigned short, h);
+  float r;
+  asm("v_fma_mix_f32 %0, %1, -1.0, %2 op_sel_hi:[1,0,0]" : "=v"(r) : "v"(hb), "v"(x));
+  l = (hx_t)r;
+#endif
+}
 __device__ __forceinline__ void orl_split4x3(const f32x4& v, hx4& h, hx4& m, hx4& l) {
   h = __builtin_convertvector(v, hx4);
 #if defined(ORL_SPLIT_BF16) || defined(ORL_SPLIT_NO_MIX)
diff --git a/offlinerl-kit_amd/csrc/ws_debug.hip b/offlinerl-kit_amd/csrc/ws_debug.hip
--- a/offlinerl-kit_amd/csrc/ws_debug.hip
+++ b/offlinerl-kit_amd/csrc/ws_debug.hip
@@ -86,7 +86,7 @@
     const orl_gemm_buf& b = *bufs[i];
     const std::string name = WS_BUF_NAMES[i];
     if (!b.host) { why = name + " is required"; return false; }
-    if (b.n <= 0 || b.n > (1L << 28)) { why = name + ": bad element count"; return false; }
+    if (b.n <= 0 || (b.n > (1L << 28) && !a->dry_run)) { why = name + ": bad element count"; return false; }
     if (b.off < 0 || b.s0 < 0 || b.s1 < 0 || b.ks < 0 || b.pitch < 0) { why = name + ": negative offset, pitch or stride"; return false; }
     if (ext < 1) { why = name + ": empty extent"; return false; }
     if (result && ((nz0 > 1 && b.s0 < ext) || (nz1 > 1 && b.s1 < ext) || (nslab > 1 && b.ks < ext))) { why = name + ": problems or slabs of a result overlap"; return false; }
diff --git a/offlinerl-kit_amd/csrc/ws_device.h b/offlinerl-kit_amd/csrc/ws_device.h
--- a/offlinerl-kit_amd/csrc/ws_device.h
+++ b/offlinerl-kit_amd/csrc/ws_device.h
@@ -22,6 +22,15 @@
 __device__ __forceinline__ void ws_split8(const f32x4& a, const f32x4& b, hx8 (&pl)[2]) { ws_split8(a, b, pl[0], pl[1]); }
 __device__ __forceinline__ void ws_split8(const f32x4& a, const f32x4& b, hx8 (&pl)[3]) { ws_split8x3(a, b, pl[0], pl[1], pl[2]); }
 
+template <class T, class B>
+__device__ __forceinline__ __attribute__((address_space(1))) T& ws_g(B* ubase, unsigned int& lane_bytes, int imm_bytes = 0) {
+  asm("" : "+v"(lane_bytes));
+  typedef __attribute__((address_space(1))) char* gptr;
+  return *(__attribute__((address_space(1))) T*)((gptr)const_cast<void*>((const void*)ubase) + (size_t)lane_bytes + imm_bytes);
+}
+template <class B>
+__device__ __forceinline__ char* ws_lb(B* region, unsigned int bytes) { return (char*)const_cast<void*>((const void*)region) + bytes; }
+
 __device__ __forceinline__ int ws_a_off(int r, int kq) { return r * WS_PITCH + ((((kq >> 1) ^ (r & 15)) << 3) | ((kq & 1) << 2)); }
 __device__ __forceinline__ int ws_a_frag(int s, int li, int c) { return (16 * s + li) * WS_PITCH + ((c ^ li) << 3); }
 
@@ -83,6 +92,39 @@
 __device__ __forceinline__ void ws_x_load(const float* __restrict__ X0g, int g, int xe, int tid, float (&sx)[XI]) {
 #pragma unroll
   for (int i = 0; i < XI; ++i) { const int e = tid + WS_NT * i; sx[i] = X0g[(long)g * xe + (e < xe ? e : xe - 1)]; }
+}
+template <int XI>
+__device__ __forceinline__ void ws_x_offsets(bool on, int tid, int xe, unsigned int (&vo)[XI]) {
+#pragma unroll
+  for (int i = 0; i < XI; ++i) { const int e = tid + WS_NT * i; vo[i] = on ? 4u * (unsigned int)(e < xe ? e : xe - 1) : 0u; }
+}
+template <int XI>
+__device__ __forceinline__ void ws_x_load(const float* __restrict__ X0g, int g, int xe, unsigned int (&vo)[XI], float (&sx)[XI]) {
+#pragma unroll
+  for (int i = 0; i < XI; ++i) sx[i] = ws_g<const float>(X0g + (long)g * xe, vo[i]);
+}
+template <int XLP, int XI, int NP>
+__device__ __forceinline__ void ws_x_slots(const int (&xr)[XI], const int (&xc)[XI], unsigned int (&la)[XI][NP]) {
+#pragma unroll
+  for (int i = 0; i < XI; ++i) {
+    const bool pad = xc[i] >= 32;
+    if constexpr (NP == 1) la[i][0] = (unsigned int)(xr[i] * XLP + xc[i]) * 4u;
+    else { la[i][0] = (unsigned int)(xr[i] * XLP * 4 + 2 * (pad ? 64 : xc[i])); la[i][1] = (unsigned int)(xr[i] * XLP * 4 + 2 * (pad ? 65 : 32 + xc[i])); }
+  }
+}
+template <int XI, int NP>
+__device__ __forceinline__ void ws_x_store_at(char* xl, int in0, const int (&xc)[XI], const unsigned int (&la)[XI][NP], const float (&sx)[XI]) {
+#pragma unroll
+  for (int i = 0; i < XI; ++i) {
+    const float x = (xc[i] == in0) ? 1.0f : sx[i];
+    if constexpr (NP == 1) *(float*)(xl + la[i][0]) = x;
+    else {
+      hx_t hh, ll;
+      orl_split1m(x, hh, ll);
+      *(hx_t*)(xl + la[i][0]) = hh;
+      *(hx_t*)(xl + la[i][1]) = ll;
+    }
+  }
 }
 template <int NPL, int XLP, int XI>
 __device__ __forceinline__ void ws_x_store(float* Xl, int buf, int in0, const int (&xr)[XI], const int (&xc)[XI], const float (&sx)[XI]) {
diff --git a/offlinerl-kit_amd/csrc/ws_dgrad.hip b/offlinerl-kit_amd/csrc/ws_dgrad.hip
--- a/offlinerl-kit_amd/csrc/ws_dgrad.hip
+++ b/offlinerl-kit_amd/csrc/ws_dgrad.hip
@@ -59,6 +59,7 @@
   float sx[2];
   const int xe = W0 ? WS_ROWS * p.x_pitch : 0;
   float* __restrict__ Cg = STORE ? p.C.p + z0 * p.C.s0 + z1 * p.C.s1 : nullptr;
+  unsigned int vo_c = STORE ? 4u * (unsigned int)(4 * lq * p.c_pitch + ncol0 + li) : 0u;
   int xo[2];
 #pragma unroll
   for (int i = 0; i < 2; ++i) {
@@ -70,25 +71,29 @@
   float sdq;
   unsigned int sxw;
   f32x4 sz[PLAIN ? 4 : 1];
-  const unsigned int vo_z = PLAIN ? (unsigned int)((tid >> 6) * p.z_pitch + 4 * (tid & 63)) : 0u;
-  const unsigned int vo_ab = (unsigned int)((tid >> 4) * p.ab_g + ((tid & 15) >> 1)), vo_dq = (unsigned int)((tid & 31) * (int)p.dq_sm);
-  const unsigned int vo_xb = (unsigned int)(((tid >> 3) & 31) * p.xb_g + (tid & 7));
+  unsigned int vo_z = PLAIN ? 4u * (unsigned int)((tid >> 6) * p.z_pitch + 4 * (tid & 63)) : 0u;
+  unsigned int vo_ab = 4u * (unsigned int)((tid >> 4) * p.ab_g + ((tid & 15) >> 1)), vo_dq = 4u * (unsigned int)((tid & 31) * (int)p.dq_sm);
+  unsigned int vo_xb = 4u * (unsigned int)(((tid >> 3) & 31) * p.xb_g + (tid & 7));
   unsigned int vo_x[2];
 #pragma unroll
-  for (int i = 0; i < 2; ++i) { const int e = tid + WS_NT * i; vo_x[i] = (unsigned int)(e < xe ? e : (xe > 0 ? xe - 1 : 0)); }
+  for (int i = 0; i < 2; ++i) { const int e = tid + WS_NT * i; vo_x[i] = 4u * (unsigned int)(e < xe ? e : (xe > 0 ? xe - 1 : 0)); }
+  constexpr unsigned int A_BUF = APL * WS_ROWS * WS_PITCH * 2, A_SUB = 16 * WS_PITCH * 2, XT_BUF = 2 * 32 * WD_XP * 2, EO_BUF = (WS_ROWS + WS_NW * WS_ROWS) * 4;
+  const unsigned int la_f = (unsigned int)ws_a_frag(0, li, lq) * 2u;
+  const unsigned int la_e = 16u * lq, la_w = (unsigned int)(WS_ROWS + wave * WS_ROWS + 4 * lq) * 4u;
+  const unsigned int la_x = (unsigned int)(li * WD_XP + 4 * lq) * 2u;
   auto load_group = [&](int g) __attribute__((always_inline)) {
     const long row0 = (long)g * WS_ROWS;
     if (PLAIN) {
 #pragma unroll
-      for (int i = 0; i < 4; ++i) sz[i] = *(const f32x4*)&(Zg + (row0 + 8 * i) * p.z_pitch)[vo_z];
+      for (int i = 0; i < 4; ++i) sz[i] = ws_g<const f32x4>(Zg + (row0 + 8 * i) * p.z_pitch, vo_z);
     } else {
-      sm_word = (ab + row0 * p.ab_g)[vo_ab];
-      sdq = (dqg + row0 * p.dq_sm)[vo_dq];
-    }
-    sxw = (xb + row0 * p.xb_g)[vo_xb];
+      sm_word = ws_g<const unsigned int>(ab + row0 * p.ab_g, vo_ab);
+      sdq = ws_g<const float>(dqg + row0 * p.dq_sm, vo_dq);
+    }
+    sxw = ws_g<const unsigned int>(xb + row0 * p.xb_g, vo_xb);
     if (W0) {
 #pragma unroll
-      for (int i = 0; i < 2; ++i) sx[i] = (Xg + (long)g * xe)[vo_x[i]];
+      for (int i = 0; i < 2; ++i) sx[i] = ws_g<const float>(Xg + (long)g * xe, vo_x[i]);
     }
   };
   auto store_group = [&](int buf) __attribute__((always_inline)) {
@@ -123,7 +128,7 @@
       if (W0) {
         const float x = (xo[i] >> 16) ? 1.0f : sx[i];
         hx_t hh, ll;
-        orl_split1(x, hh, ll);
+        orl_split1m(x, hh, ll);
         xt[xo[i] & 0xFFFF] = hh;
         xt[32 * WD_XP + (xo[i] & 0xFFFF)] = ll;
       }
@@ -147,15 +152,15 @@
     const int buf = it & 1;
     f32x4 dq4[WS_SUB];
     unsigned int xw[WS_SUB][4];
-    const float* eo = EO + buf * (WS_ROWS + WS_NW * WS_ROWS);
+    const char* eo = ws_lb(EO, buf * EO_BUF);
 #pragma unroll
     for (int s = 0; s < WS_SUB; ++s) {
-      dq4[s] = PLAIN ? (f32x4){1.f, 1.f, 1.f, 1.f} : *(const f32x4*)&eo[16 * s + 4 * lq];
-      const u32x4 w4 = *(const u32x4*)&((const unsigned int*)eo)[WS_ROWS + wave * WS_ROWS + 16 * s + 4 * lq];
+      dq4[s] = PLAIN ? (f32x4){1.f, 1.f, 1.f, 1.f} : *(const f32x4*)(eo + la_e + 64 * s);
+      const u32x4 w4 = *(const u32x4*)(eo + la_w + 64 * s);
 #pragma unroll
       for (int r = 0; r < 4; ++r) xw[s][r] = w4[r];
     }
-    const hx_t* ah = Ah + (long)buf * APL * WS_ROWS * WS_PITCH;
+    const unsigned int ab_l = la_f + buf * A_BUF;
     f32x4 acc[WS_SUB][2];
 #pragma unroll
     for (int s = 0; s < WS_SUB; ++s)
@@ -165,9 +170,10 @@
     for (int ks = 0; ks < 8; ++ks) {
 #pragma unroll
       for (int s = 0; s < WS_SUB; ++s) {
-        const hx8 fa = *(const hx8*)&ah[(16 * s + li) * WS_PITCH + (((4 * ks + lq) ^ li) << 3)];
+        const char* a = ws_lb(Ah, s * A_SUB + (ks >> 2) * 256) + (ab_l ^ (unsigned int)(64 * (ks & 3)));
+        const hx8 fa = *(const hx8*)a;
         hx8 fl;
-        if (PLAIN) fl = *(const hx8*)&ah[WS_ROWS * WS_PITCH + (16 * s + li) * WS_PITCH + (((4 * ks + lq) ^ li) << 3)];
+        if (PLAIN) fl = *(const hx8*)(a + WS_ROWS * WS_PITCH * 2);
 #pragma unroll
         for (int cb = 0; cb < 2; ++cb) {
           acc[s][cb] = ORL_MFMA_16x16x32(fa, bl[cb][ks], acc[s][cb]);
@@ -176,16 +182,15 @@
         }
       }
     }
-    const hx_t* xth = XT + (long)buf * 2 * 32 * WD_XP;
-    const hx_t* xtl = xth + 32 * WD_XP;
+    const char* xt = ws_lb(XT, buf * XT_BUF) + la_x;
 #pragma unroll
     for (int s = 0; s < WS_SUB; ++s) {
       s16x4 xh[2], xl[2];
       if (W0) {
 #pragma unroll
         for (int cbk = 0; cbk < 2; ++cbk) {
-          xh[cbk] = *(const s16x4*)&xth[(16 * cbk + li) * WD_XP + 16 * s + 4 * lq];
-          xl[cbk] = *(const s16x4*)&xtl[(16 * cbk + li) * WD_XP + 16 * s + 4 * lq];
+          xh[cbk] = *(const s16x4*)(xt + (16 * cbk * WD_XP * 2 + 32 * s));
+          xl[cbk] = *(const s16x4*)(xt + (32 * WD_XP * 2 + 16 * cbk * WD_XP * 2 + 32 * s));
         }
       }
 #pragma unroll
@@ -194,9 +199,9 @@
 #pragma unroll
         for (int r = 0; r < 4; ++r) {
           const float v = ((xw[s][r] >> (16 * cb + li)) & 1u) ? (PLAIN ? acc[s][cb][r] : acc[s][cb][r] * dq4[s][r]) : 0.f;
-          if (STORE) Cg[(long)(g * WS_ROWS + 16 * s + 4 * lq + r) * p.c_pitch + ncol0 + 16 * cb + li] = v;
+          if (STORE) ws_g<float>(Cg + ((long)g * WS_ROWS + 16 * s + r) * p.c_pitch, vo_c, 64 * cb) = v;
           hx_t hh, ll;
-          orl_split1(v, hh, ll);
+          orl_split1m(v, hh, ll);
           zh[r] = hh; zl[r] = ll;
         }
         const s16x4 bzh = *(const s16x4*)&zh, bzl = *(const s16x4*)&zl;
@@ -416,6 +421,7 @@
 }
 
 hipError_t launch_ws_dgrad_w0(WsDgradP p, int nz, int per_z, hipStream_t st) {
+  if (!ws_dgrad_span32(p)) return hipErrorInvalidValue;
   p.groups = p.M / WS_ROWS;
   static const hipError_t attr_err = ws_table_attrs(ws_dgrad_table());
   if (attr_err != hipSuccess) return attr_err;
diff --git a/offlinerl-kit_amd/csrc/ws_fwd.hip b/offlinerl-kit_amd/csrc/ws_fwd.hip
--- a/offlinerl-kit_amd/csrc/ws_fwd.hip
+++ b/offlinerl-kit_amd/csrc/ws_fwd.hip
@@ -27,6 +27,14 @@
   const int ncol0 = 16 * WS_CB * wave;
   float* __restrict__ Y0g = L0 ? const_cast<float*>(Xg) : nullptr;
   const float* __restrict__ X0g = L0 ? p.X0.p + z0 * p.X0.s0 + z1 * p.X0.s1 : nullptr;
+  unsigned int vo_st, vo_h0, vo_y, vo_dm, vo_mb, vo_mb0, vo_tq;
+  unsigned int la_f, la_p, la_nb, la_q, la_xf;
+  unsigned int* __restrict__ mbg = DG ? nullptr : p.mb.p + z0 * p.mb.s0 + z1 * p.mb.s1;
+  unsigned int* __restrict__ mb0g = L0 ? p.mb0.p + z0 * p.mb0.s0 + z1 * p.mb0.s1 : nullptr;
+  float* __restrict__ tqg = TQ ? p.tq.p + z0 * p.tq.s0 + z1 * p.tq.s1 : nullptr;
+  constexpr unsigned int A_BUF = F32 ? WS_ROWS * WS_K * 4 : 2 * WS_ROWS * WS_PITCH * 2, A_LO = WS_ROWS * WS_PITCH * 2;
+  constexpr unsigned int A_SUB = F32 ? 16 * WS_K * 4 : 16 * WS_PITCH * 2;
+  constexpr unsigned int NB_PAR = WS_ROWS * WS_NBP, Q_PAR = WS_NW * WS_ROWS * 4, XL_BUF = WS_ROWS * WS_XLP * 4;
 
   WS_STAMP(0);
   hx8 bh[WS_CB][F32 ? 1 : 8], bl[WS_CB][F32 ? 1 : 8];
@@ -75,9 +83,7 @@
 
   f32x4 st0[WS_LD];
   auto load_piece = [&](int g, f32x4 (&st)[WS_LD], int i) __attribute__((always_inline)) {
-    const int idx = tid + WS_NT * i, r = idx >> 6, kq = idx & 63;
-    int m = g * WS_ROWS + r; m = m < p.M ? m : p.M - 1;
-    st[i] = *(const f32x4*)&Xg[(long)m * p.x_pitch + 4 * kq];
+    st[i] = ws_g<const f32x4>(Xg + ((long)g * WS_ROWS + (WS_NT / 64) * i) * p.x_pitch, vo_st);
   };
   auto load_group = [&](int g, f32x4 (&st)[WS_LD]) __attribute__((always_inline)) {
 #pragma unroll
@@ -105,33 +111,30 @@
   constexpr int XI = (WS_ROWS * 32 + WS_NT - 1) / WS_NT;
   int xr[XI], xc[XI];
   float sx[XI];
-  ws_x_index(L0, tid, p.x0_pitch, xe, xr, xc);
-  auto loadX = [&](int g) __attribute__((always_inline)) { ws_x_load(X0g, g, xe, tid, sx); };
-  auto storeX = [&](int buf) __attribute__((always_inline)) { ws_x_store<F32 ? 0 : 2, WS_XLP>(Xl, buf, p.in0, xr, xc, sx); };
+  unsigned int vo_x0[XI], la_xs[XI][F32 ? 1 : 2];
+  auto loadX = [&](int g) __attribute__((always_inline)) { ws_x_load(X0g, g, xe, vo_x0, sx); };
+  auto storeX = [&](int buf) __attribute__((always_inline)) { ws_x_store_at(ws_lb(Xl, buf * XL_BUF), p.in0, xc, la_xs, sx); };
   f32x4 fx32[2];
   auto prod_x = [&](int xbuf, int s, hx8 (&xa)[2]) __attribute__((always_inline)) {
-    if constexpr (F32) ws_x_frag<WS_XLP>(Xl, xbuf, s, li, lq, fx32); else ws_x_frag<WS_XLP>(Xl, xbuf, s, li, lq, xa);
+    const char* xp = ws_lb(Xl, xbuf * XL_BUF) + la_xf + s * (16 * WS_XLP * 4);
+    if constexpr (F32) { fx32[0] = *(const f32x4*)xp; fx32[1] = *(const f32x4*)(xp + 64); } else { xa[0] = *(const hx8*)xp; xa[1] = *(const hx8*)(xp + 64); }
   };
   auto prod_block = [&](int g, int buf, int par, int s, int cb, const hx8 (&xa)[2]) __attribute__((always_inline)) {
-    hx_t* dh = Ah + (long)buf * 2 * WS_ROWS * WS_PITCH;
-    hx_t* dl = dh + WS_ROWS * WS_PITCH;
-    const int r = 16 * s + li;
-    const long m = (long)g * WS_ROWS + r;
     f32x4 v;
     unsigned int nib0;
     if constexpr (F32) nib0 = ws_h0_block(b0w[cb], fx32, v); else nib0 = ws_h0_block(b0[cb], xa, v);
-    const int k = ncol0 + 16 * cb + 4 * lq;
-    if constexpr (XS) *(f32x4*)&Y0g[m * p.x_pitch + k] = v;
+    if constexpr (XS) ws_g<f32x4>(Y0g + ((long)g * WS_ROWS + 16 * s) * p.x_pitch, vo_h0, 64 * cb) = v;
+    static_assert(WS_CB <= 4 && WS_NW * WS_CB == 16, "the column block occupies its own bits of the chunk index");
+    char* d = ws_lb(ws_smem, s * A_SUB) + ((la_p + buf * A_BUF) ^ (unsigned int)((F32 ? 64 : 32) * cb));
     if constexpr (F32) {
-      *(f32x4*)(Af + (long)buf * WS_ROWS * WS_K + r * WS_K + (((k >> 2) ^ (r & 15)) << 2)) = v;
+      *(f32x4*)d = v;
     } else {
     hx4 h, l;
     orl_split4(v, h, l);
-    const int o = ws_a_off(r, k >> 2);
-    *(hx4*)(dh + o) = h;
-    *(hx4*)(dl + o) = l;
-    }
-    nbs0[(par * WS_ROWS + r) * WS_NBP + (k >> 2)] = (unsigned char)nib0;
+    *(hx4*)d = h;
+    *(hx4*)(d + A_LO) = l;
+    }
+    *(unsigned char*)(ws_lb(nbs0, par * NB_PAR) + la_nb + (16 * s * WS_NBP + 4 * cb)) = (unsigned char)nib0;
   };
   auto produce = [&](int g, int buf, int xbuf, int par) __attribute__((always_inline)) {
 #pragma unroll
@@ -146,12 +149,31 @@
     if (tid < WS_ROWS * 8) {
       const int row = tid >> 3, wd = tid & 7;
       const unsigned int word = ws_pack_nibbles(nbs0 + (par * WS_ROWS + row) * WS_NBP + 8 * wd);
-      p.mb0.p[z0 * p.mb0.s0 + z1 * p.mb0.s1 + ((long)g * WS_ROWS + row) * p.mb0_g + wd] = word;
+      ws_g<unsigned int>(mb0g + (long)g * WS_ROWS * p.mb0_g, vo_mb0) = word;
     }
   };
 
   const int g0 = blockIdx.x, gs = gridDim.x;
   if (g0 >= p.groups) return;
+  auto set_addr = [&](int t) __attribute__((always_inline)) {
+    const int tid = t, wave = tid >> 6, lane = tid & 63, li = lane & 15, lq = lane >> 4, ncol0 = 16 * WS_CB * wave;
+    vo_st = (unsigned int)((tid >> 6) * p.x_pitch + 4 * (tid & 63)) * 4u;
+    vo_h0 = (unsigned int)(li * p.x_pitch + ncol0 + 4 * lq) * 4u;
+    vo_y = (unsigned int)(li * p.y_pitch + ncol0 + 4 * lq) * 4u;
+    vo_dm = DG ? (unsigned int)(li * p.dm_g + (ncol0 >> 5)) * 4u : 0u;
+    vo_mb = (unsigned int)((tid >> 3) * p.mb_g + (tid & 7)) * 4u;
+    vo_mb0 = L0 ? (unsigned int)((tid >> 3) * p.mb0_g + (tid & 7)) * 4u : 0u;
+    vo_tq = TQ ? (unsigned int)tid * (unsigned int)p.tq_sm * 4u : 0u;
+    la_f = F32 ? (unsigned int)(li * WS_K + ((lq ^ li) << 2)) * 4u : (unsigned int)ws_a_frag(0, li, lq) * 2u;
+    la_p = !L0 ? 0u : (F32 ? (unsigned int)(li * WS_K + ((((ncol0 + 4 * lq) >> 2) ^ li) << 2)) * 4u : (unsigned int)ws_a_off(li, (ncol0 + 4 * lq) >> 2) * 2u);
+    la_nb = (unsigned int)(li * WS_NBP + 4 * WS_CB * wave + lq);
+    la_q = (unsigned int)(wave * WS_ROWS + li) * 4u;
+    la_xf = (unsigned int)(li * WS_XLP * 4 + 16 * lq);
+    ws_x_index(L0, tid, p.x0_pitch, xe, xr, xc);
+    ws_x_offsets(L0, tid, xe, vo_x0);
+    ws_x_slots<WS_XLP>(xr, xc, la_xs);
+  };
+  set_addr(tid);
   WS_STAMP(2);
   if (L0) {
     for (int e = tid; e < 2 * WS_ROWS * WS_XLP; e += WS_NT) Xl[e] = 0.f;
@@ -174,18 +196,17 @@
   constexpr bool storeY = SY;
   auto epi_block = [&](const f32x4& a, int g, int par, int s, int cb, float& part) __attribute__((always_inline)) {
     const f32x4 bq = *(const f32x4*)&cst[ncol0 + 16 * cb + 4 * lq], twq = *(const f32x4*)&cst[WS_N + ncol0 + 16 * cb + 4 * lq];
-    const int m = g * WS_ROWS + 16 * s + li;
     f32x4 v = F32 ? a + bq : a * inv_sc + bq;
     const unsigned int nib = orl_relu_mask4(v);
-    if (storeY) *(f32x4*)&Yg[(long)m * p.y_pitch + ncol0 + 16 * cb + 4 * lq] = v;
+    if (storeY) ws_g<f32x4>(Yg + ((long)g * WS_ROWS + 16 * s) * p.y_pitch, vo_y, 64 * cb) = v;
     part += (v[0] * twq[0] + v[1] * twq[1]) + (v[2] * twq[2] + v[3] * twq[3]);
-    nbs[(par * WS_ROWS + 16 * s + li) * WS_NBP + 4 * WS_CB * wave + 4 * cb + lq] = (unsigned char)nib;
+    *(unsigned char*)(ws_lb(nbs, par * NB_PAR) + la_nb + (16 * s * WS_NBP + 4 * cb)) = (unsigned char)nib;
   };
   auto epi_row = [&](int par, int s, float part) __attribute__((always_inline)) {
     if (TQ) {
       part += __shfl_xor(part, 16);
       part += __shfl_xor(part, 32);
-      (qs + (par * WS_NW + wave) * WS_ROWS)[16 * s + li] = part;
+      *(float*)(ws_lb(qs, par * Q_PAR) + la_q + 64 * s) = part;
     }
   };
   auto epilogue = [&](const f32x4 (&acc)[WS_SUB][WS_CB], int g, int par) __attribute__((always_inline)) {
@@ -193,15 +214,15 @@
       const unsigned int* __restrict__ dm = p.dmask.p + z0 * p.dmask.s0 + z1 * p.dmask.s1;
 #pragma unroll
       for (int s = 0; s < WS_SUB; ++s) {
-        const long m = (long)g * WS_ROWS + 16 * s + li;
-        const unsigned int w = dm[m * p.dm_g + (ncol0 >> 5)];
+        const long m0 = (long)g * WS_ROWS + 16 * s;
+        const unsigned int w = ws_g<const unsigned int>(dm + m0 * p.dm_g, vo_dm);
 #pragma unroll
         for (int cb = 0; cb < WS_CB; ++cb) {
           const unsigned int nib = w >> ((ncol0 & 31) + 16 * cb + 4 * lq);
           f32x4 v = acc[s][cb];
 #pragma unroll
           for (int r = 0; r < 4; ++r) v[r] = ((nib >> r) & 1u) ? (F32 ? v[r] : v[r] * inv_sc) : 0.f;
-          *(f32x4*)&Yg[m * p.y_pitch + ncol0 + 16 * cb + 4 * lq] = v;
+          ws_g<f32x4>(Yg + m0 * p.y_pitch, vo_y, 64 * cb) = v;
         }
       }
       return;
@@ -217,22 +238,20 @@
   auto finish = [&](int g, int par) __attribute__((always_inline)) {
     if (DG) return;
     if (tid < WS_ROWS * 8) {
-      const int row = tid >> 3, wd = tid & 7, m = g * WS_ROWS + row;
+      const int row = tid >> 3, wd = tid & 7;
       const unsigned int word = ws_pack_nibbles(nbs + (par * WS_ROWS + row) * WS_NBP + 8 * wd);
-      p.mb.p[z0 * p.mb.s0 + z1 * p.mb.s1 + (long)m * p.mb_g + wd] = word;
+      ws_g<unsigned int>(mbg + (long)g * WS_ROWS * p.mb_g, vo_mb) = word;
     }
     if (TQ && tid < WS_ROWS) {
-      const int m = g * WS_ROWS + tid;
       const float q = ws_tail_sum(qs + par * WS_NW * WS_ROWS + tid, tbias);
-      p.tq.p[z0 * p.tq.s0 + z1 * p.tq.s1 + (long)m * p.tq_sm] = q;
+      ws_g<float>(tqg + (long)g * WS_ROWS * p.tq_sm, vo_tq) = q;
     }
   };
 
   f32x4 pacc[WS_SUB][WS_CB];
   auto iteration = [&](int g, int it, f32x4 (&stn)[WS_LD], bool first, bool steady) __attribute__((always_inline)) {
     const int buf = it & 1;
-    const hx_t* ah = Ah + (long)buf * 2 * WS_ROWS * WS_PITCH;
-    const hx_t* al = ah + WS_ROWS * WS_PITCH;
+    const unsigned int ab = la_f + buf * A_BUF;
     f32x4 acc[WS_SUB][WS_CB];
 #pragma unroll
     for (int s = 0; s < WS_SUB; ++s)
@@ -299,12 +318,11 @@
 #pragma unroll
     for (int ks = 0; ks < 8; ++ks) {
       if constexpr (F32) {
-        const float* af = Af + (long)buf * WS_ROWS * WS_K;
 #pragma unroll
         for (int tt = 0; tt < 2; ++tt) {
           f32x4 fa[WS_SUB];
 #pragma unroll
-          for (int s = 0; s < WS_SUB; ++s) fa[s] = *(const f32x4*)&af[(16 * s + li) * WS_K + (((8 * ks + 4 * tt + lq) ^ li) << 2)];
+          for (int s = 0; s < WS_SUB; ++s) fa[s] = *(const f32x4*)(ws_lb(ws_smem, s * A_SUB + ((2 * ks + tt) >> 2) * 256) + (ab ^ (unsigned int)(64 * ((2 * ks + tt) & 3))));
 #pragma unroll
           for (int e = 0; e < 4; ++e)
 #pragma unroll
@@ -317,8 +335,8 @@
       hx8 fah2[WS_SUB], fal2[WS_SUB];
 #pragma unroll
       for (int s = 0; s < WS_SUB; ++s) {
-        const int o = ws_a_frag(s, li, 4 * ks + lq);
-        fah2[s] = *(const hx8*)&ah[o]; fal2[s] = *(const hx8*)&al[o];
+        const char* a = ws_lb(ws_smem, s * A_SUB + (ks >> 2) * 256) + (ab ^ (unsigned int)(64 * (ks & 3)));
+        fah2[s] = *(const hx8*)a; fal2[s] = *(const hx8*)(a + A_LO);
       }
 #pragma unroll
       for (int s = 0; s < WS_SUB; ++s)
@@ -361,6 +379,11 @@
   };
   int g = g0, it = 0;
   WS_STAMP(3);
+  {
+    int t = tid;
+    asm("" : "+v"(t));
+    set_addr(t);
+  }
   iteration(g, it, st0, true, false);
   WS_STAMP(4);
   g += gs; ++it;
@@ -402,6 +425,7 @@
 }
 
 hipError_t launch_ws_fwd(WsFwdP p, int nz, hipStream_t st, const WsGeom& geo) {
+  if (!ws_fwd_span32(p)) return hipErrorInvalidValue;
   p.groups = (p.M + WS_ROWS - 1) / WS_ROWS;
   const int per_z = ws_blocks_per_problem(p.groups, nz, 10, 1 << 20, geo);
   static const hipError_t attr_err = ws_table_attrs(ws_fwd_table());
diff --git a/offlinerl-kit_amd/csrc/ws_gemm.h b/offlinerl-kit_amd/csrc/ws_gemm.h
--- a/offlinerl-kit_amd/csrc/ws_gemm.h
+++ b/offlinerl-kit_amd/csrc/ws_gemm.h
@@ -84,10 +84,17 @@
   return best;
 }
 
+static inline bool ws_span32(long pitch) { return pitch >= 0 && (unsigned long)pitch * WS_ROWS * 4 <= 0xFFFFFFFFul; }
+static inline bool ws_fwd_span32(const WsFwdP& p) {
+  return ws_span32(p.x_pitch) && (!p.Y.p || ws_span32(p.y_pitch)) && (!p.mb.p || ws_span32(p.mb_g)) && (!p.mb0.p || ws_span32(p.mb0_g)) &&
+         (!p.tq.p || ws_span32(p.tq_sm)) && (!p.dmask.p || ws_span32(p.dm_g));
+}
+
 const WsTable& ws_fwd_table();
 int ws_fwd_flavour(const WsFwdP& p);
 static inline bool ws_fwd_supported(const WsFwdP& p, int K, int N) {
   if (K != WS_K || N != WS_N || p.M < 256 || (p.M % WS_ROWS) || (!p.mb.p && !p.dmask.p)) return false;
+  if (!ws_fwd_span32(p)) return false;
   if (!p.X.vec4() || (p.x_pitch & 3)) return false;
   if (p.w_sk == 1 && (!p.W.vec4() || (p.w_sn & 3))) return false;
   if (p.dmask.p) { if (p.tq.p || p.X0.p || p.dm_g != 8) return false; }
@@ -142,8 +149,12 @@
 
 const WsTable& ws_dgrad_table();
 int ws_dgrad_flavour(const WsDgradP& p);
+static inline bool ws_dgrad_span32(const WsDgradP& p) {
+  return ws_span32(p.ab_g) && ws_span32(p.xb_g) && ws_span32(p.dq_sm) && (!p.Z.p || ws_span32(p.z_pitch)) && (!p.C.p || ws_span32(p.c_pitch)) && ws_span32(p.x_pitch);
+}
 static inline bool ws_dgrad_supported(const WsDgradP& p, int K, int N) {
   if (K != WS_K || N != WS_N || p.M < 256 || (p.M % WS_ROWS)) return false;
+  if (!ws_dgrad_span32(p)) return false;
   if (p.Z.p) {
     if (!p.w0_out || p.C.p || !p.xbits.p || p.xb_g != 8) return false;
     if (!p.Z.vec4() || (p.z_pitch & 3)) return false;
@@ -202,7 +213,11 @@
 
 const WsTable& ws_wgrad_table();
 int ws_wgrad_flavour(const WsWgradP& p);
+static inline bool ws_wgrad_span32(const WsWgradP& p) {
+  return ws_span32(p.ab_g) && ws_span32(p.dq_sm) && (!p.H0.p || ws_span32(p.h0_pitch)) && (!p.H1.p || ws_span32(p.h1_pitch)) && (!p.dZ.p || ws_span32(p.dz_pitch));
+}
 static inline bool ws_wgrad_supported(const WsWgradP& p, int K, int N) {
+  if (!ws_wgrad_span32(p)) return false;
   if (p.dZ.p) {
     if (K != WS_K || N != WS_N || p.M < 256 || (p.M % WS_ROWS)) return false;
     if (!p.dZ.vec4() || (p.dz_pitch & 3)) return false;
diff --git a/offlinerl-kit_amd/csrc/ws_wgrad.hip b/offlinerl-kit_amd/csrc/ws_wgrad.hip
--- a/offlinerl-kit_amd/csrc/ws_wgrad.hip
+++ b/offlinerl-kit_amd/csrc/ws_wgrad.hip
@@ -9,6 +9,12 @@
   const hx_t* a = img + ww_off(row, col >> 3, (col >> 2) & 1);
   return __builtin_amdgcn_ds_read_tr16_b64_v4i16((s16x4 __attribute__((address_space(3)))*)a);
 }
+
+__device__ inline unsigned int ww_tr_lane(int lane) {
+  const int li = lane & 15, lq = lane >> 4;
+  return (unsigned int)ww_off(4 * lq + (li >> 2), (li & 3) >> 1, li & 1) * 2u;
+}
+__device__ inline s16x4 ww_trb(const char* a) { return __builtin_amdgcn_ds_read_tr16_b64_v4i16((s16x4 __attribute__((address_space(3)))*)a); }
 
 template <int MODE>
 __device__ __forceinline__ void ww_finish(const WsWgradP& p, float* ws_smem, const f32x4 (&acc)[16][2], const f32x4 (&accb)[2], const f32x4& tacc,
@@ -192,18 +198,19 @@
     *(hx4*)(gh + o) = h;
     *(hx4*)(gl + o) = l;
   };
-  const unsigned int vo_h0 = (unsigned int)((tid >> 6) * p.h0_pitch + 4 * (tid & 63));
-  const unsigned int vo_h1 = (TAILS || PLAIN) ? (unsigned int)((tid >> 6) * h1_pitch + 4 * (tid & 63)) : 0u;
-  const unsigned int vo_dq = (unsigned int)((tid >> 6) * (int)p.dq_sm);
-  const unsigned int vo_ab = (unsigned int)((tid >> 4) * p.ab_g + ((tid & 15) >> 1));
+  unsigned int vo_h0 = 4u * (unsigned int)((tid >> 6) * p.h0_pitch + 4 * (tid & 63));
+  unsigned int vo_h1 = (TAILS || PLAIN) ? 4u * (unsigned int)((tid >> 6) * h1_pitch + 4 * (tid & 63)) : 0u;
+  unsigned int vo_dq = 4u * (unsigned int)((tid >> 6) * (int)p.dq_sm);
+  unsigned int vo_ab = 4u * (unsigned int)((tid >> 4) * p.ab_g + ((tid & 15) >> 1));
+  const unsigned int la_t = ww_tr_lane(lane), la_tw = la_t ^ (unsigned int)(64 * wave);
   auto load_piece = [&](int g, int i) __attribute__((always_inline)) {
     const long row0 = (long)g * WS_ROWS + 8 * i;
-    if (!RECOMP) s0[i] = *(const f32x4*)&(H0g + row0 * p.h0_pitch)[vo_h0];
-    if (TAILS || PLAIN) s1[i] = *(const f32x4*)&(H1g + row0 * h1_pitch)[vo_h1];
-    if (!PLAIN) sdq[i] = (dqg + row0 * p.dq_sm)[vo_dq];
+    if (!RECOMP) s0[i] = ws_g<const f32x4>(H0g + row0 * p.h0_pitch, vo_h0);
+    if (TAILS || PLAIN) s1[i] = ws_g<const f32x4>(H1g + row0 * h1_pitch, vo_h1);
+    if (!PLAIN) sdq[i] = ws_g<const float>(dqg + row0 * p.dq_sm, vo_dq);
   };
   auto load_mask = [&](int g) __attribute__((always_inline)) {
-    if (!PLAIN) sm_word = (ab + (long)g * WS_ROWS * p.ab_g)[vo_ab];
+    if (!PLAIN) sm_word = ws_g<const unsigned int>(ab + (long)g * WS_ROWS * p.ab_g, vo_ab);
   };
   auto load_group = [&](int g) __attribute__((always_inline)) {
     load_mask(g);
@@ -322,20 +329,25 @@
         *(s16x4*)&r = x; *((s16x4*)&r + 1) = y;
         return r;
       };
+      const unsigned int ta = la_t + buf * (NPL * WW_IMG * 2), tb = la_tw + buf * (NPL * WW_IMG * 2);
+      auto tr2 = [&](const hx_t* plane, unsigned int t, int kb) __attribute__((always_inline)) {
+        const char* a = ws_lb(plane - (long)buf * NPL * WW_IMG, 0) + (t ^ (unsigned int)(32 * kb));
+        return cat(ww_trb(a), ww_trb(a + 16 * WS_K * 2));
+      };
       hx8 bh[2], bl[2], bm[2];
 #pragma unroll
       for (int nb = 0; nb < 2; ++nb) {
-        bh[nb] = cat(ww_tr(gh, 0, ncol0 + 16 * nb, lane), ww_tr(gh, 16, ncol0 + 16 * nb, lane));
-        bl[nb] = cat(ww_tr(gl, 0, ncol0 + 16 * nb, lane), ww_tr(gl, 16, ncol0 + 16 * nb, lane));
-        if (P3) bm[nb] = cat(ww_tr(gm, 0, ncol0 + 16 * nb, lane), ww_tr(gm, 16, ncol0 + 16 * nb, lane));
+        bh[nb] = tr2(gh, tb, nb);
+        bl[nb] = tr2(gl, tb, nb);
+        if (P3) bm[nb] = tr2(gm, tb, nb);
       }
       const int dro0 = (4 * lq + (li >> 2)) * 16 + 4 * (li & 3), dro1 = dro0 + 16 * 16;
       typedef s16x4 __attribute__((address_space(3))) * lds_s16x4;
 #pragma unroll
       for (int kp = 0; kp < 8; ++kp) {
         const int kb0 = 2 * kp, kb1 = kb0 + 1;
-        const hx8 a0 = cat(ww_tr(mi, 0, 16 * kb0, lane), ww_tr(mi, 16, 16 * kb0, lane));
-        const hx8 a1 = cat(ww_tr(mi, 0, 16 * kb1, lane), ww_tr(mi, 16, 16 * kb1, lane));
+        const hx8 a0 = tr2(mi, ta, kb0);
+        const hx8 a1 = tr2(mi, ta, kb1);
 #pragma unroll
         for (int nb = 0; nb < 2; ++nb) acc[kb0][nb] = ORL_MFMA_16x16x32(a0, bl[nb], acc[kb0][nb]);
 #pragma unroll
@@ -347,8 +359,8 @@
           for (int nb = 0; nb < 2; ++nb) acc[kb1][nb] = ORL_MFMA_16x16x32(a1, bm[nb], acc[kb1][nb]);
         }
         if (PLAIN) {
-          const hx8 l0 = cat(ww_tr(ml, 0, 16 * kb0, lane), ww_tr(ml, 16, 16 * kb0, lane));
-          const hx8 l1 = cat(ww_tr(ml, 0, 16 * kb1, lane), ww_tr(ml, 16, 16 * kb1, lane));
+          const hx8 l0 = tr2(ml, ta, kb0);
+          const hx8 l1 = tr2(ml, ta, kb1);
 #pragma unroll
           for (int nb = 0; nb < 2; ++nb) acc[kb0][nb] = ORL_MFMA_16x16x32(l0, bh[nb], acc[kb0][nb]);
 #pragma unroll
@@ -365,11 +377,11 @@
                     __builtin_amdgcn_ds_read_tr16_b64_v4i16((lds_s16x4)(dqi + (DQP - 1) * WS_ROWS * 16 + dro1)));
           if (P3) bdm = cat(__builtin_amdgcn_ds_read_tr16_b64_v4i16((lds_s16x4)(dqi + WS_ROWS * 16 + dro0)),
                             __builtin_amdgcn_ds_read_tr16_b64_v4i16((lds_s16x4)(dqi + WS_ROWS * 16 + dro1)));
-          const hx8 c0 = cat(ww_tr(mi, 0, 32 * wave, lane), ww_tr(mi, 16, 32 * wave, lane));
-          const hx8 c1 = cat(ww_tr(mi, 0, 32 * wave + 16, lane), ww_tr(mi, 16, 32 * wave + 16, lane));
+          const hx8 c0 = tr2(mi, tb, 0);
+          const hx8 c1 = tr2(mi, tb, 1);
           if (PLAIN) {
-            const hx8 e0 = cat(ww_tr(ml, 0, 32 * wave, lane), ww_tr(ml, 16, 32 * wave, lane));
-            const hx8 e1 = cat(ww_tr(ml, 0, 32 * wave + 16, lane), ww_tr(ml, 16, 32 * wave + 16, lane));
+            const hx8 e0 = tr2(ml, tb, 0);
+            const hx8 e1 = tr2(ml, tb, 1);
             accb[0] = ORL_MFMA_16x16x32(e0, bdh, accb[0]);
             accb[1] = ORL_MFMA_16x16x32(e1, bdh, accb[1]);
           } else {
@@ -618,6 +630,7 @@
 }
 
 hipError_t launch_ws_wgrad(WsWgradP p, int nz, int per_z, hipStream_t st) {
+  if (!ws_wgrad_span32(p)) return hipErrorInvalidValue;
   p.groups = p.M / WS_ROWS;
   static const hipError_t attr_err = ws_table_attrs(ws_wgrad_table());
   if (attr_err != hipSuccess) return attr_err;
```

Result: faster. 55870 (median of 6 runs) (+2.5%).
